# jzbontar/mc-cnn

Hardware: AMD Instinct MI355X
Metric: Mega-pixel-disparities/sec (cost-vol+CBCA+SGM) + end-to-end disp ms/pair (higher is better)
Workload: dtype f32; 1 GPU; KITTI 2012 fast, 370x1226 disp_max=228; H=370, W=1226, disp_max=228, feature_channels=64, params=kitti_fast, parallelism=one pair per GPU

## Files before the change

mc-cnn_amd/csrc/api.hip:

```cpp
#include "cbca_common.h"

#include <stdarg.h>
#include <algorithm>
#include <map>
#include <mutex>
#include <vector>

namespace mc {

int fill_nan(float *p, int64_t n, hipStream_t st);
int scale(const float *in, float *out, int64_t n, float s, hipStream_t st);
int transpose(const float *in, float *out, int64_t R, int64_t Cn, int64_t ldin, int64_t ldout, float s, hipStream_t st, int nt = -1);
int fix_border(float *vol, int D, int H, int W, int n, int direction, hipStream_t st);
int argmin_dhw(const float *vol, float *out, int D, int H, int W, int base1, hipStream_t st);
int outlier_detection(const float *d0, const float *d1, float *outlier, int H, int W, int disp_max, hipStream_t st);
int interpolate_occlusion(const float *d0, const float *outlier, float *out, int H, int W, hipStream_t st);
int interpolate_mismatch(const float *d0, const float *outlier, float *out, int H, int W, hipStream_t st);
int subpixel(const float *d0, const float *vol, float *out, int D, int H, int W, int64_t sd, int64_t sp, hipStream_t st);
int median2d(const float *img, float *out, int H, int W, int k, hipStream_t st);
int mean2d(const float *img, const float *kernel, float *out, int H, int W, int ks, float alpha2, hipStream_t st);
int normalize_forward(const float *in, float *norm, float *out, int N, int C, int H, int W, hipStream_t st);
int stereo_join_dhw(const float *fL, const float *fR, float *volL, float *volR, int C, int D, int H, int W, hipStream_t st);
int stereo_join_hwd(const float *fL, const float *fR, float *volL, float *volR, int C, int D, int ds, int H, int W, int n,
                    hipStream_t st);
int ad_tiled(const float *x0, const float *x1, float *vol, int D, int H, int W, int direction, hipStream_t st);
size_t census_scratch_bytes(int Cimg, int H, int W);
int census_sig(const float *x0, const float *x1, float *vol, void *scratch, int Cimg, int D, int H, int W, int direction,
               hipStream_t st);
int cross(const float *img, float *arms, int H, int W, int L1, float tau1, hipStream_t st);
int cbca(const float *x0c, const float *x1c, const float *vin, float *vout, int D, int H, int W, int direction, hipStream_t st);
size_t cbca_scratch_bytes(int H, int W);
int cbca_pack(const float *x0c, const float *x1c, void *scratch, int H, int W, hipStream_t st);
int cbca_if_overflow(const float *x0c, const float *x1c, const void *packed, const float *vin, float *vout, int D, int H, int W,
                     int direction, hipStream_t st);
int cbca_strips(const void *packed, const float *vin, float *vout, int D, int H, int W, int direction, int route,
               hipStream_t st, const CbcaCfg &cfg = CbcaCfg());
size_t cbca_plan_bytes(int D, int H, int W);
int cbca_tiles(const void *packed, const float *vin, float *vout, int D, int H, int W, int direction, int arm_class, int route,
               hipStream_t st, const CbcaCfg &cfg = CbcaCfg());
bool cbca_lean_fits(int D, int H, int W, size_t plan_bytes, bool two_pass = false, int rb = 0);
int cbca_classify(const void *packed, void *plan, size_t plan_bytes, int D, int H, int W, int direction, int route, int rb, int cap_limit,
                  hipStream_t st, bool two_pass = false, float cost_limit = 0);
int cbca_lean2x(const void *packed, const void *plan, size_t plan_bytes, const float *vin, float *vout, int D, int H, int W, int direction,
                int route, hipStream_t st, const CbcaCfg &cfg);
int cbca_lean(const void *packed, const void *plan, size_t plan_bytes, const float *vin, float *vout, int D, int H, int W, int direction,
              int route, hipStream_t st, const CbcaCfg &cfg);
size_t conv3x3_workspace_bytes(int Cin, int Cout);
int conv3x3(const float *in, const float *w, const float *bias, float *out, int N, int Cin, int Cout, int H, int W, int relu,
            void *workspace, hipStream_t st);
size_t fc_workspace_bytes(int C, int n_hidden, int H, int W);
int fc_stack(const float *featL, const float *featR, int C, int H, int W, int D, const float *const *weights,
             const float *const *biases, int n_layers, float *volL, float *volR, void *workspace, hipStream_t st);
size_t sgm_maps_bytes(int H, int W);
int sgm_prep(const float *x0, const float *x1, void *maps, int H, int W, float tau_so, hipStream_t st);
int sgm_contract_violations(const float *vol, int H, int W, int D, unsigned *count, hipStream_t st);
int sgm_sweeps(const float *const C[2], float *const out[2], float *const out2[2], float *const disp[2],
               const int direction[2], int nvol, int H, int W, int D, int ds, const void *maps, float pi1, float pi2,
               float alpha1, float q1, float q2, bool fused, unsigned drop_final, hipStream_t st);

static thread_local char g_err[512] = "";

void set_error(const char *fmt, ...)
{
	va_list ap;
	va_start(ap, fmt);
	vsnprintf(g_err, sizeof(g_err), fmt, ap);
	va_end(ap);
}

int check_launch(const char *what)
{
	const hipError_t e = hipPeekAtLastError();
	if (e != hipSuccess) {
		(void)hipGetLastError();
		set_error("%s: %s", what, hipGetErrorString(e));
		return (int)e;
	}
	return 0;
}

static bool dims_ok(int D, int H, int W) { return D >= 1 && H >= 1 && W >= 1 && (int64_t)D * H * W < ((int64_t)1 << 40); }

static void gaussian_fill(double sigma, float *k)
{
	const int kr = (int)ceil(sigma * 3);
	const int ks = kr * 2 + 1;
	for (int i = 1; i <= ks; ++i) {
		for (int j = 1; j <= ks; ++j) {
			const double y = (i - 1) - kr;
			const double x = (j - 1) - kr;
			k[(size_t)(i - 1) * ks + (j - 1)] = (float)exp(-(x * x + y * y) / (2 * sigma * sigma));
		}
	}
}
struct GaussianK { const float *data; size_t n; };
static int gaussian_cached(double sigma, GaussianK &out)
{
	static std::mutex mu;
	static std::map<double, GaussianK> cache;
	std::lock_guard<std::mutex> lk(mu);
	auto it = cache.find(sigma);
	if (it != cache.end()) { out = it->second; return 0; }
	const int kr = (int)ceil(sigma * 3);
	const int ks = kr * 2 + 1;
	float *k = nullptr;
	const hipError_t e = hipHostMalloc((void **)&k, (size_t)ks * ks * sizeof(float), hipHostMallocDefault);
	if (e != hipSuccess) {
		set_error("gaussian: hipHostMalloc: %s", hipGetErrorString(e));
		return (int)e;
	}
	gaussian_fill(sigma, k);
	out = GaussianK{k, (size_t)ks * ks};
	cache[sigma] = out;
	return 0;
}

static inline size_t align_up(size_t v, size_t a) { return (v + a - 1) / a * a; }

static inline bool packed_dims_ok(int H, int W)
{
	return (int64_t)H * W < ((int64_t)1 << 29) - 4096 && H < (1 << 23) - 64 && W < (1 << 23) - 256;
}

static int cbca_by_arms(const void *packed, const float *vin, float *vout, int D, int H, int W, int direction, int max_arm, hipStream_t st,
                        const CbcaCfg &cfg = CbcaCfg())
{
	if (max_arm >= 0 && max_arm <= 4) return cbca_tiles(packed, vin, vout, D, H, W, direction, 4, -1, st, cfg);
	if (cfg.planned) {
		int rc = cbca_tiles(packed, vin, vout, D, H, W, direction, 13, CR_PLANNED_TILE13, st, cfg);
		if (rc || cfg.lean_two_pass) return rc;
		return cbca_strips(packed, vin, vout, D, H, W, direction, CR_STRIP_IF_LIST, st, cfg);
	}
	int rc = cbca_tiles(packed, vin, vout, D, H, W, direction, 4, CR_TILE4, st, cfg);
	if (rc) return rc;
	if (max_arm < 0 || max_arm <= 13) {
		rc = cbca_tiles(packed, vin, vout, D, H, W, direction, 13, CR_TILE13, st, cfg);
		if (rc) return rc;
	}
	if (cfg.lean) {
		if (!cfg.lean_two_pass) {
			rc = cbca_lean(packed, cfg.plan, cfg.plan_bytes, vin, vout, D, H, W, direction, CR_STRIP, st, cfg);
			if (rc) return rc;
		}
		return cbca_strips(packed, vin, vout, D, H, W, direction, CR_STRIP_IF_NO_LIST, st, cfg);
	}
	return cbca_strips(packed, vin, vout, D, H, W, direction, max_arm > 13 ? CR_STRIP_OR_TILE13 : CR_STRIP, st, cfg);
}

struct Plan {
	int Dp;
	size_t maps, arms, pack, vol, img, gk;
	size_t cplan;
	int nplan;
	size_t total;
};

struct StageCounts { int cbca1, sgm, cbca2; bool active_after; };
static StageCounts stage_counts(const mc_params *p)
{
	StageCounts c;
	bool sm_active = p->sm_terminate != MC_SM_CNN;
	c.cbca1 = (sm_active && p->sm_skip != MC_SKIP_CBCA) ? p->cbca_i1 : 0;
	sm_active = sm_active && p->sm_terminate != MC_SM_CBCA1;
	c.sgm = (sm_active && p->sm_skip != MC_SKIP_SGM) ? p->sgm_i : 0;
	sm_active = sm_active && p->sm_terminate != MC_SM_SGM;
	c.cbca2 = (sm_active && p->sm_skip != MC_SKIP_CBCA) ? p->cbca_i2 : 0;
	sm_active = sm_active && p->sm_terminate != MC_SM_CBCA2;
	c.active_after = sm_active;
	return c;
}

static Plan make_plan(const mc_params *p, int D, int H, int W)
{
	Plan pl;
	pl.Dp = (D + 3) / 4 * 4;
	const size_t HW = (size_t)H * W;
	pl.maps = align_up(sgm_maps_bytes(H, W), 256);
	pl.arms = align_up(8 * HW * sizeof(float), 256);
	pl.pack = cbca_scratch_bytes(H, W);
	pl.vol = align_up((size_t)pl.Dp * HW * sizeof(float), 256);
	pl.img = align_up(HW * sizeof(float), 256);
	const int kr = (int)ceil(p->blur_sigma * 3);
	const int ks = 2 * kr + 1;
	pl.gk = align_up((size_t)ks * ks * sizeof(float), 256);
	const StageCounts sc = stage_counts(p);
	pl.cplan = (sc.cbca1 + sc.cbca2 >= 2 && p->L1 - 1 <= 13) ? align_up(cbca_plan_bytes(D, H, W), 256) : 0;
	pl.nplan = (p->left_only && !p->lr_check) ? 1 : 2;
	constexpr int NVOLS = 6;
	pl.total = pl.maps + pl.arms + pl.pack + NVOLS * pl.vol + 6 * pl.img + pl.gk + pl.nplan * pl.cplan;
	return pl;
}

struct StageTimer {
	bool on = false;
	hipStream_t st;
	std::vector<hipEvent_t> ev;
	std::vector<int> tag;
	void mark(int stage)
	{
		if (!on) return;
		hipEvent_t e;
		(void)hipEventCreate(&e);
		(void)hipEventRecord(e, st);
		ev.push_back(e);
		tag.push_back(stage);
	}
	void collect(float out[MC_N_STAGES])
	{
		for (int i = 0; i < MC_N_STAGES; ++i) out[i] = 0;
		if (!on || ev.empty()) return;
		(void)hipEventSynchronize(ev.back());
		for (size_t i = 1; i < ev.size(); ++i) {
			float ms = 0;
			(void)hipEventElapsedTime(&ms, ev[i - 1], ev[i]);
			if (tag[i] >= 0 && tag[i] < MC_N_STAGES) out[tag[i]] += ms;
		}
		for (auto e : ev) (void)hipEventDestroy(e);
		ev.clear();
	}
};
enum { ST_PREP = MC_STAGE_PREP, ST_JOIN = MC_STAGE_JOIN, ST_CBCA = MC_STAGE_CBCA, ST_LAYOUT = MC_STAGE_LAYOUT,
       ST_SGM = MC_STAGE_SGM, ST_ARGMIN = MC_STAGE_ARGMIN, ST_POST = MC_STAGE_POST };

static int predict_impl(const mc_params *p, const float *x0, const float *x1, const float *featL, const float *featR, int C,
                        const float *rawL, const float *rawR, int D, int H, int W, void *workspace, size_t workspace_bytes,
                        float *volL_out, float *volR_out, float *dispL0_out, float *dispR0_out, float *disp_out, hipStream_t st,
                        StageTimer &tm)
{
	MC_REQUIRE(p && x0 && x1 && disp_out && workspace, "mc_predict: null argument");
	MC_REQUIRE(dims_ok(D, H, W), "mc_predict: bad dims D=%d H=%d W=%d", D, H, W);
	MC_REQUIRE(D <= MC_SGM_MAX_D, "mc_predict: D=%d exceeds %d", D, MC_SGM_MAX_D);
	MC_REQUIRE((featL && featR && C >= 1) || (rawL && rawR), "mc_predict: need features or raw volumes");
	MC_REQUIRE(p->cbca_i1 >= 0 && p->cbca_i2 >= 0 && p->sgm_i >= 0, "mc_predict: negative iteration count");
	MC_REQUIRE(p->median_k % 2 == 1 && p->median_k <= 11, "mc_predict: median_k must be odd and <= 11");
	MC_REQUIRE(p->blur_sigma > 0, "mc_predict: blur_sigma must be > 0");
	MC_REQUIRE(p->sm_terminate >= 0 && p->sm_terminate <= MC_SM_BILATERAL && p->sm_skip >= 0 && p->sm_skip <= MC_SKIP_BILATERAL,
	           "mc_predict: bad sm_terminate / sm_skip");
	const bool from_feat = featL != nullptr;
	if (from_feat) MC_REQUIRE(p->border_n >= 0 && p->border_n < W, "mc_predict: border_n=%d out of range", p->border_n);
	if (from_feat) MC_REQUIRE(C <= MC_JOIN_MAX_C, "mc_predict: C=%d exceeds %d (adcensus.cu:1460)", C, MC_JOIN_MAX_C);
	const Plan pl = make_plan(p, D, H, W);
	MC_REQUIRE(workspace_bytes >= pl.total, "mc_predict: workspace %zu < %zu bytes", workspace_bytes, pl.total);
	MC_REQUIRE((uintptr_t)workspace % 256 == 0, "mc_predict: workspace must be 256-byte aligned");

	const int64_t HW = (int64_t)H * W;
	const int64_t V = (int64_t)D * HW;
	char *w = (char *)workspace;
	void *maps = w; w += pl.maps;
	float *x0c = (float *)w; float *x1c = x0c + 4 * HW; w += pl.arms;
	void *packed = w; w += pl.pack;
	float *bufA[2], *bufB[2];
	bufA[0] = (float *)w; w += pl.vol;
	bufA[1] = (float *)w; w += pl.vol;
	bufB[0] = (float *)w; w += pl.vol;
	bufB[1] = (float *)w; w += pl.vol;
	float *bufC[2];
	bufC[0] = (float *)w; w += pl.vol;
	bufC[1] = (float *)w; w += pl.vol;
	float *img[6];
	for (int i = 0; i < 6; ++i) { img[i] = (float *)w; w += pl.img; }
	float *gk = (float *)w; w += pl.gk;
	void *cplan[2] = {pl.cplan ? (void *)w : nullptr, (pl.cplan && pl.nplan > 1) ? (void *)(w + pl.cplan) : nullptr};
	int cplan_passes[2] = {0, 0};
	bool cplan_listed[2] = {false, false};
	const int Dp = pl.Dp;
	int rc;
#define RUN(call) do { rc = (call); if (rc) return rc; } while (0)

	const int direction[2] = {-1, 1};
	const StageCounts sc = stage_counts(p);
	const int n_cbca1 = sc.cbca1, n_sgm = sc.sgm, n_cbca2 = sc.cbca2;
	bool sm_active = sc.active_after;
	const bool use_cbca = (n_cbca1 + n_cbca2) > 0;
	tm.mark(-1);

	if (n_sgm > 0) RUN(sgm_prep(x0, x1, maps, H, W, p->tau_so, st));
	if (use_cbca) {
		RUN(cross(x0, x0c, H, W, p->L1, p->tau1, st));
		RUN(cross(x1, x1c, H, W, p->L1, p->tau1, st));
		RUN(cbca_pack(x0c, x1c, packed, H, W, st));
	}
	const int cbca_cap = p->L1 - 1;
	tm.mark(ST_PREP);

	const int ds = Dp;
	const float *cur[2];
	auto other = [&](int v) -> float * { return cur[v] == bufA[v] ? bufB[v] : bufA[v]; };
	bool hwd;
	const int nvol = (p->left_only && !p->lr_check && !volR_out && !dispR0_out) ? 1 : 2;
	auto cbca_iterations = [&](int n) -> int {
		const bool packed_ok = cbca_cap <= 254 && packed_dims_ok(H, W);
		for (int v = 0; v < nvol; ++v) {
			const bool planned = packed_ok && cplan[v] && cbca_cap > 4 && cbca_cap <= 13 && cbca_lean_fits(D, H, W, pl.cplan, true);
			if (planned && n > 0 && !cplan_listed[v]) {
				const int rc1 = cbca_classify(packed, cplan[v], pl.cplan, D, H, W, direction[v], CR_STRIP, 0, 0, st, true);
				if (rc1) return rc1;
				cplan_listed[v] = true;
			}
			for (int i = 0; i < n;) {
				float *dst = other(v);
				CbcaCfg cfg;
				cfg.plan = cplan[v];
				cfg.plan_bytes = pl.cplan;
				cfg.planned = planned;
				const bool two = planned && i + 1 < n;
				cfg.lean = cfg.lean_two_pass = two;
				float *mid = two ? bufC[v] : dst;
				for (int half = 0; half < (two ? 2 : 1); ++half) {
					cfg.plan_mode = cplan[v] ? (cplan_passes[v]++ == 0 ? 1 : 2) : 0;
					const float *src = half == 0 ? cur[v] : mid;
					float *to = (two && half == 0) ? mid : dst;
					const int rc2 = packed_ok ? cbca_by_arms(packed, src, to, D, H, W, direction[v], cbca_cap, st, cfg)
					                          : cbca(x0c, x1c, src, to, D, H, W, direction[v], st);
					if (rc2) return rc2;
				}
				if (two) {
					const int rc3 = cbca_lean2x(packed, cplan[v], pl.cplan, cur[v], dst, D, H, W, direction[v], CR_STRIP, st, cfg);
					if (rc3) return rc3;
				}
				cur[v] = dst;
				i += two ? 2 : 1;
			}
		}
		return 0;
	};
	const bool join_fits = (int64_t)W * ((D + 3) / 4 * 4) * 4 < ((int64_t)1 << 31) && ((int64_t)(C + 64) * HW + W) * 4 < ((int64_t)1 << 31);
	if (from_feat && n_cbca1 == 0 && n_sgm > 0 && join_fits) {
		RUN(stereo_join_hwd(featL, featR, bufA[0], bufA[1], C, D, ds, H, W, p->border_n, st));
		cur[0] = bufA[0]; cur[1] = bufA[1];
		hwd = true;
		tm.mark(ST_JOIN);
	} else {
		if (from_feat) {
			RUN(fill_nan(bufA[0], V, st));
			RUN(fill_nan(bufA[1], V, st));
			RUN(stereo_join_dhw(featL, featR, bufA[0], bufA[1], C, D, H, W, st));
			RUN(fix_border(bufA[0], D, H, W, p->border_n, -1, st));
			RUN(fix_border(bufA[1], D, H, W, p->border_n, 1, st));
			cur[0] = bufA[0]; cur[1] = bufA[1];
		} else {
			cur[0] = rawL; cur[1] = rawR;
		}
		hwd = false;
		tm.mark(ST_JOIN);
		RUN(cbca_iterations(n_cbca1));
		tm.mark(ST_CBCA);
	}

	float *dispv[2] = {img[0], img[1]};
	bool have_disp = false;
	if (n_sgm > 0) {
		if (!hwd) {
			for (int v = 0; v < nvol; ++v) {
				float *dst = other(v);
				RUN(transpose(cur[v], dst, D, HW, HW, ds, 1.0f, st));
				cur[v] = dst;
			}
			hwd = true;
			tm.mark(ST_LAYOUT);
		}
		for (int it = 0; it < n_sgm; ++it) {
			const float *Cv[2] = {cur[0], cur[1]};
			float *outv[2] = {other(0), other(1)};
			const bool am = (it == n_sgm - 1) && n_cbca2 == 0;
			const unsigned drop_final = (am && nvol == 2 && !volR_out) ? 2u : 0u;
			RUN(sgm_sweeps(Cv, outv, bufC, am ? dispv : nullptr, direction, nvol, H, W, D, ds, maps, p->pi1, p->pi2, p->alpha1,
			               p->sgm_q1, p->sgm_q2, true, drop_final, st));
			have_disp = am;
			cur[0] = outv[0]; cur[1] = outv[1];
		}
		tm.mark(ST_SGM);
		if (n_cbca2 > 0) {
			for (int v = 0; v < nvol; ++v) {
				float *dst = other(v);
				RUN(transpose(cur[v], dst, HW, D, ds, HW, 1.0f, st));
				cur[v] = dst;
			}
			hwd = false;
			tm.mark(ST_LAYOUT);
		}
	}
	if (!hwd) {
		RUN(cbca_iterations(n_cbca2));
		tm.mark(ST_CBCA);
	}

	MC_REQUIRE(have_disp || !hwd, "mc_predict: an (H,W,D) volume without its arg-min");
	if (!have_disp) {
		for (int v = 0; v < nvol; ++v) RUN(argmin_dhw(cur[v], dispv[v], D, H, W, 0, st));
	}
	float *vout[2] = {volL_out, volR_out};
	for (int v = 0; v < nvol; ++v) {
		if (!vout[v]) continue;
		if (hwd) RUN(transpose(cur[v], vout[v], HW, D, ds, HW, 1.0f, st));
		else RUN(scale(cur[v], vout[v], V, 1.0f, st));
	}
	if (dispL0_out) RUN(scale(dispv[0], dispL0_out, HW, 1.0f, st));
	if (dispR0_out) RUN(scale(dispv[1], dispR0_out, HW, 1.0f, st));
	tm.mark(ST_ARGMIN);

	float *d = dispv[0];
	float *outl = img[4];
	int nfree = 0;
	float *freeimg[3] = {img[2], img[3], img[5]};
	auto next = [&]() -> float * {
		float *r = freeimg[nfree % 3];
		if (r == d) r = freeimg[++nfree % 3];
		++nfree;
		return r;
	};
	if (p->lr_check) {
		RUN(outlier_detection(d, dispv[1], outl, H, W, D, st));
		if (sm_active && p->sm_skip != MC_SKIP_OCCLUSION) {
			float *o = next();
			RUN(interpolate_occlusion(d, outl, o, H, W, st));
			d = o;
		}
		sm_active = sm_active && p->sm_terminate != MC_SM_OCCLUSION;
		if (sm_active && p->sm_skip != MC_SKIP_OCCLUSION) {
			float *o = next();
			RUN(interpolate_mismatch(d, outl, o, H, W, st));
			d = o;
		}
		sm_active = sm_active && p->sm_terminate != MC_SM_MISMATCH;
	}
	if (sm_active && p->sm_skip != MC_SKIP_SUBPIXEL) {
		float *o = next();
		if (hwd) RUN(subpixel(d, cur[0], o, D, H, W, 1, ds, st));
		else RUN(subpixel(d, cur[0], o, D, H, W, HW, 1, st));
		d = o;
	}
	sm_active = sm_active && p->sm_terminate != MC_SM_SUBPIXEL;
	if (sm_active && p->sm_skip != MC_SKIP_MEDIAN) {
		float *o = next();
		RUN(median2d(d, o, H, W, p->median_k, st));
		d = o;
	}
	sm_active = sm_active && p->sm_terminate != MC_SM_MEDIAN;
	if (sm_active && p->sm_skip != MC_SKIP_BILATERAL) {
		GaussianK k;
		RUN(gaussian_cached(p->blur_sigma, k));
		const int ks = 2 * (int)ceil(p->blur_sigma * 3) + 1;
		const hipError_t e = hipMemcpyAsync(gk, k.data, k.n * sizeof(float), hipMemcpyHostToDevice, st);
		if (e != hipSuccess) {
			set_error("mc_predict: kernel upload: %s", hipGetErrorString(e));
			return (int)e;
		}
		RUN(mean2d(d, gk, disp_out, H, W, ks, p->blur_t, st));
	} else {
		RUN(scale(d, disp_out, HW, 1.0f, st));
	}
	tm.mark(ST_POST);
#undef RUN
	return 0;
}

}

using namespace mc;

extern "C" {

int mc_version(void) { return MC_ABI_VERSION; }
const char *mc_last_error(void) { return g_err; }

int mc_fill_nan(float *p, int64_t n, void *stream)
{
	MC_REQUIRE(p || n == 0, "mc_fill_nan: null pointer");
	MC_REQUIRE(n >= 0, "mc_fill_nan: negative size");
	return fill_nan(p, n, as_stream(stream));
}

int mc_stereo_join(const float *featL, const float *featR, float *volL, float *volR, int C, int D, int H, int W, void *stream)
{
	MC_REQUIRE(featL && featR && volL && volR, "mc_stereo_join: null pointer");
	MC_REQUIRE(dims_ok(D, H, W) && C >= 1, "mc_stereo_join: bad dims C=%d D=%d H=%d W=%d", C, D, H, W);
	MC_REQUIRE(C <= MC_JOIN_MAX_C, "mc_stereo_join: C=%d exceeds %d (adcensus.cu:1460)", C, MC_JOIN_MAX_C);
	MC_REQUIRE(D <= 65535, "mc_stereo_join: D too large");
	return stereo_join_dhw(featL, featR, volL, volR, C, D, H, W, as_stream(stream));
}

int mc_ad(const float *x0, const float *x1, float *vol, int D, int H, int W, int direction, void *stream)
{
	MC_REQUIRE(x0 && x1 && vol, "mc_ad: null pointer");
	MC_REQUIRE(dims_ok(D, H, W), "mc_ad: bad dims");
	MC_REQUIRE(direction == -1 || direction == 1, "mc_ad: direction must be -1 or 1");
	MC_REQUIRE(D <= 65535, "mc_ad: D too large");
	return ad_tiled(x0, x1, vol, D, H, W, direction, as_stream(stream));
}

size_t mc_census_scratch_bytes(int Cimg, int H, int W)
{
	if (Cimg < 1 || H < 1 || W < 1) return 0;
	return census_scratch_bytes(Cimg, H, W);
}

int mc_census_ws(const float *x0, const float *x1, float *vol, int Cimg, int D, int H, int W, int direction, void *scratch,
                 size_t scratch_bytes, void *stream)
{
	MC_REQUIRE(x0 && x1 && vol && scratch, "mc_census_ws: null pointer");
	MC_REQUIRE(dims_ok(D, H, W) && Cimg >= 1 && D <= 65535, "mc_census_ws: bad dims");
	MC_REQUIRE(direction == -1 || direction == 1, "mc_census_ws: direction must be -1 or 1");
	MC_REQUIRE(scratch_bytes >= census_scratch_bytes(Cimg, H, W), "mc_census_ws: scratch holds %zu bytes, needs %zu", scratch_bytes,
	           census_scratch_bytes(Cimg, H, W));
	MC_REQUIRE((uintptr_t)scratch % 4 == 0, "mc_census_ws: scratch must be 4-byte aligned");
	return census_sig(x0, x1, vol, scratch, Cimg, D, H, W, direction, as_stream(stream));
}

size_t mc_fc_stack_workspace_bytes(int C, int n_layers, int H, int W)
{
	if (C < 1 || n_layers < 2 || n_layers > 8 || H < 1 || W < 1) return 0;
	return fc_workspace_bytes(C, n_layers - 2, H, W);
}

int mc_fc_stack(const float *featL, const float *featR, int C, int H, int W, int D, const float *const *weights,
                const float *const *biases, const int *layer_out, int n_layers, float *volL, float *volR, void *workspace,
                size_t workspace_bytes, void *stream)
{
	MC_REQUIRE(featL && featR && weights && biases && layer_out && volL && volR && workspace, "mc_fc_stack: null pointer");
	MC_REQUIRE(dims_ok(D, H, W) && C >= 1, "mc_fc_stack: bad dims");
	MC_REQUIRE(n_layers >= 2 && n_layers <= 8, "mc_fc_stack: 2..8 layers supported");
	for (int l = 0; l < n_layers - 1; ++l)
		MC_REQUIRE(layer_out[l] == 384, "mc_fc_stack: hidden width %d not supported (nh2 = 384 in every preset, main.lua:77,124)",
		           layer_out[l]);
	MC_REQUIRE(layer_out[n_layers - 1] == 1, "mc_fc_stack: the last layer must have one output");
	for (int l = 0; l < n_layers; ++l) MC_REQUIRE(weights[l] && biases[l], "mc_fc_stack: null layer %d", l);
	MC_REQUIRE(workspace_bytes >= fc_workspace_bytes(C, n_layers - 2, H, W), "mc_fc_stack: workspace %zu < %zu bytes",
	           workspace_bytes, fc_workspace_bytes(C, n_layers - 2, H, W));
	MC_REQUIRE((uintptr_t)workspace % 16 == 0, "mc_fc_stack: workspace must be 16-byte aligned");
	MC_REQUIRE((int64_t)((H + 7) / 8) * ((W + 95) / 96) * D * 8 < ((int64_t)1 << 31), "mc_fc_stack: problem too large for one launch");
	return fc_stack(featL, featR, C, H, W, D, weights, biases, n_layers, volL, volR, workspace, as_stream(stream));
}

size_t mc_conv3x3_workspace_bytes(int Cin, int Cout)
{
	if (Cin < 1 || Cout < 1 || Cout > 128) return 0;
	return conv3x3_workspace_bytes(Cin, Cout);
}

int mc_conv3x3(const float *in, const float *weight, const float *bias, float *out, int N, int Cin, int Cout, int H, int W,
               int relu, void *workspace, size_t workspace_bytes, void *stream)
{
	MC_REQUIRE(in && weight && bias && out && workspace && in != out, "mc_conv3x3: bad pointers");
	MC_REQUIRE(N >= 1 && Cin >= 1 && Cout >= 1 && dims_ok(1, H, W), "mc_conv3x3: bad dims");
	MC_REQUIRE(Cout <= 128, "mc_conv3x3: Cout=%d exceeds 128 (the nets of main.lua:73-75, 120-122 use 64 and 112)", Cout);
	MC_REQUIRE((int64_t)(Cout > Cin ? Cout : Cin + 1) * H * W * 4 < (int64_t)0xFFFFFF00 && (int64_t)N * ((W + 31) / 32) * H < ((int64_t)1 << 31),
	           "mc_conv3x3: %d x %d x (%d -> %d channels) x %d images exceeds the kernel's 32-bit offsets", H, W, Cin, Cout, N);
	MC_REQUIRE(workspace_bytes >= conv3x3_workspace_bytes(Cin, Cout), "mc_conv3x3: workspace %zu < %zu bytes", workspace_bytes,
	           conv3x3_workspace_bytes(Cin, Cout));
	MC_REQUIRE((uintptr_t)workspace % 16 == 0, "mc_conv3x3: workspace must be 16-byte aligned");
	return conv3x3(in, weight, bias, out, N, Cin, Cout, H, W, relu, workspace, as_stream(stream));
}

int mc_fix_border(float *vol, int D, int H, int W, int n, int direction, void *stream)
{
	MC_REQUIRE(vol, "mc_fix_border: null pointer");
	MC_REQUIRE(dims_ok(D, H, W), "mc_fix_border: bad dims");
	MC_REQUIRE(n >= 0 && n < W, "mc_fix_border: n=%d out of range for W=%d", n, W);
	MC_REQUIRE(direction == -1 || direction == 1, "mc_fix_border: direction must be -1 or 1");
	return fix_border(vol, D, H, W, n, direction, as_stream(stream));
}

int mc_cross(const float *img, float *arms, int H, int W, int L1, float tau1, void *stream)
{
	MC_REQUIRE(img && arms, "mc_cross: null pointer");
	MC_REQUIRE(dims_ok(1, H, W), "mc_cross: bad dims");
	return cross(img, arms, H, W, L1, tau1, as_stream(stream));
}

int mc_cbca(const float *x0c, const float *x1c, const float *vol_in, float *vol_out, int D, int H, int W, int direction,
            void *stream)
{
	MC_REQUIRE(x0c && x1c && vol_in && vol_out, "mc_cbca: null pointer");
	MC_REQUIRE(vol_in != vol_out, "mc_cbca: in-place aggregation is not supported (the reference uses a tmp volume too)");
	MC_REQUIRE(dims_ok(D, H, W) && D <= 65535, "mc_cbca: bad dims");
	MC_REQUIRE(direction == -1 || direction == 1, "mc_cbca: direction must be -1 or 1");
	return cbca(x0c, x1c, vol_in, vol_out, D, H, W, direction, as_stream(stream));
}

size_t mc_cbca_scratch_bytes(int H, int W)
{
	if (H < 1 || W < 1) return 0;
	return cbca_scratch_bytes(H, W);
}

int mc_cbca_ws(const float *x0c, const float *x1c, const float *vol_in, float *vol_out, int D, int H, int W, int direction,
               void *scratch, size_t scratch_bytes, void *stream)
{
	MC_REQUIRE(x0c && x1c && vol_in && vol_out && scratch, "mc_cbca_ws: null pointer");
	MC_REQUIRE(vol_in != vol_out, "mc_cbca_ws: in-place aggregation is not supported (the reference uses a tmp volume too)");
	MC_REQUIRE(dims_ok(D, H, W) && D <= 65535 * 8, "mc_cbca_ws: bad dims");
	MC_REQUIRE(direction == -1 || direction == 1, "mc_cbca_ws: direction must be -1 or 1");
	MC_REQUIRE(scratch_bytes >= cbca_scratch_bytes(H, W), "mc_cbca_ws: scratch holds %zu bytes, needs %zu", scratch_bytes,
	           cbca_scratch_bytes(H, W));
	MC_REQUIRE((uintptr_t)scratch % 4 == 0, "mc_cbca_ws: scratch must be 4-byte aligned");
	hipStream_t st = as_stream(stream);
	if (!packed_dims_ok(H, W))
		return cbca(x0c, x1c, vol_in, vol_out, D, H, W, direction, st);
	int rc = cbca_pack(x0c, x1c, scratch, H, W, st);
	if (rc) return rc;
	rc = cbca_by_arms(scratch, vol_in, vol_out, D, H, W, direction, -1, st);
	if (rc) return rc;
	return cbca_if_overflow(x0c, x1c, scratch, vol_in, vol_out, D, H, W, direction, st);
}

size_t mc_cbca_plan_bytes(int D, int H, int W)
{
	if (!dims_ok(D, H, W)) return 0;
	return align_up(cbca_scratch_bytes(H, W), 256) - cbca_scratch_bytes(H, W) + cbca_plan_bytes(D, H, W);
}

int mc_cbca_ws_cfg(const float *x0c, const float *x1c, const float *vol_in, float *vol_out, int D, int H, int W, int direction,
                   void *scratch, size_t scratch_bytes, int rb, int nt, int d0, int nd, int form, void *stream)
{
	MC_REQUIRE(x0c && x1c && vol_in && vol_out && scratch, "mc_cbca_ws_cfg: null pointer");
	MC_REQUIRE(vol_in != vol_out, "mc_cbca_ws_cfg: in-place aggregation is not supported");
	MC_REQUIRE(dims_ok(D, H, W) && D <= 65535 * 8, "mc_cbca_ws_cfg: bad dims");
	MC_REQUIRE(direction == -1 || direction == 1, "mc_cbca_ws_cfg: direction must be -1 or 1");
	MC_REQUIRE(scratch_bytes >= cbca_scratch_bytes(H, W), "mc_cbca_ws_cfg: scratch holds %zu bytes, needs %zu", scratch_bytes,
	           cbca_scratch_bytes(H, W));
	MC_REQUIRE((uintptr_t)scratch % 4 == 0, "mc_cbca_ws_cfg: scratch must be 4-byte aligned");
	MC_REQUIRE(packed_dims_ok(H, W), "mc_cbca_ws_cfg: image too large for the packed-length kernels (32-bit plane offsets, 24-bit row indices)");
	MC_REQUIRE(rb >= 0 && rb <= 4096 && nt >= -1 && nt <= 1 && form >= 0 && form <= 11, "mc_cbca_ws_cfg: bad rb / nt / form");
	MC_REQUIRE(d0 >= 0 && nd >= 0 && (form >= 8 || d0 + nd <= D), "mc_cbca_ws_cfg: planes [%d, %d) outside the volume", d0, d0 + nd);
	hipStream_t st = as_stream(stream);
	int rc = cbca_pack(x0c, x1c, scratch, H, W, st);
	if (rc) return rc;
	CbcaCfg cfg;
	cfg.nt = nt; cfg.d0 = d0; cfg.nd = nd;
	if (form >= 10) {
		const size_t off = align_up(cbca_scratch_bytes(H, W), 256), pb = align_up(cbca_plan_bytes(D, H, W), 256);
		const size_t vb = (size_t)D * H * W * sizeof(float);
		MC_REQUIRE(scratch_bytes >= off + pb + vb, "mc_cbca_ws_cfg: scratch holds %zu bytes, needs %zu with the list and a volume", scratch_bytes, off + pb + vb);
		MC_REQUIRE((uintptr_t)scratch % 16 == 0, "mc_cbca_ws_cfg: scratch must be 16-byte aligned for the list");
		cfg.plan = (char *)scratch + off;
		cfg.plan_bytes = pb;
		cfg.lean_rb = rb;
		cfg.lean_two_pass = true;
		cfg.d0 = 0; cfg.nd = 0;
		float *mid = (float *)((char *)scratch + off + pb);
		const bool fits = cbca_lean_fits(D, H, W, pb, true, rb);
		if (fits && form == 10) {
			rc = cbca_classify(scratch, cfg.plan, cfg.plan_bytes, D, H, W, direction, CR_NOT_DIRECT, rb, 0, st, true, (float)d0);
			if (rc) return rc;
		}
		if (fits) {
			rc = cbca_lean2x(scratch, cfg.plan, cfg.plan_bytes, vol_in, vol_out, D, H, W, direction, CR_NOT_DIRECT, st, cfg);
			if (rc) return rc;
		}
		const int sroute = fits ? CR_NOT_DIRECT_IF_NO_LIST : CR_NOT_DIRECT;
		rc = cbca_strips(scratch, vol_in, mid, D, H, W, direction, sroute, st, cfg);
		if (rc) return rc;
		rc = cbca_strips(scratch, mid, vol_out, D, H, W, direction, sroute, st, cfg);
		if (rc) return rc;
		rc = cbca_if_overflow(x0c, x1c, scratch, vol_in, mid, D, H, W, direction, st);
		if (rc) return rc;
		return cbca_if_overflow(x0c, x1c, scratch, mid, vol_out, D, H, W, direction, st);
	}
	if (form >= 8) {
		const size_t off = align_up(cbca_scratch_bytes(H, W), 256), pb = cbca_plan_bytes(D, H, W);
		MC_REQUIRE(scratch_bytes >= off + pb, "mc_cbca_ws_cfg: scratch holds %zu bytes, needs %zu with the list", scratch_bytes, off + pb);
		MC_REQUIRE((uintptr_t)scratch % 16 == 0, "mc_cbca_ws_cfg: scratch must be 16-byte aligned for the list");
		MC_REQUIRE(cbca_lean_fits(D, H, W, pb), "mc_cbca_ws_cfg: volume too large for 32-bit list entries");
		cfg.plan = (char *)scratch + off;
		cfg.plan_bytes = pb;
		cfg.lean_rb = rb;
		cfg.lean_variant = d0; cfg.d0 = 0; cfg.nd = nd;
		if (form == 8) {
			rc = cbca_classify(scratch, cfg.plan, cfg.plan_bytes, D, H, W, direction, CR_NOT_DIRECT, rb, nd, st);
			if (rc) return rc;
		}
		rc = cbca_lean(scratch, cfg.plan, cfg.plan_bytes, vol_in, vol_out, D, H, W, direction, CR_NOT_DIRECT, st, cfg);
		if (rc) return rc;
		cfg.nd = 0;
		rc = cbca_strips(scratch, vol_in, vol_out, D, H, W, direction, CR_NOT_DIRECT_IF_NO_LIST, st, cfg);
		if (rc) return rc;
		return cbca_if_overflow(x0c, x1c, scratch, vol_in, vol_out, D, H, W, direction, st);
	}
	if (form >= 4) {
		const size_t off = align_up(cbca_scratch_bytes(H, W), 256);
		MC_REQUIRE(scratch_bytes >= off + cbca_plan_bytes(D, H, W), "mc_cbca_ws_cfg: scratch holds %zu bytes, needs %zu with the plan", scratch_bytes,
		           off + cbca_plan_bytes(D, H, W));
		MC_REQUIRE((uintptr_t)scratch % 16 == 0, "mc_cbca_ws_cfg: scratch must be 16-byte aligned for the plan");
		cfg.plan = (char *)scratch + off;
		cfg.plan_mode = form <= 5 ? 1 : 2;
		const bool shortarm = form == 4 || form == 6;
		return cbca_tiles(scratch, vol_in, vol_out, D, H, W, direction, shortarm ? 4 : 13, shortarm ? CR_ARMS_LE4 : CR_ARMS_LE13, st, cfg);
	}
	if (form >= 2) {
		cfg.variant = rb;
		return cbca_tiles(scratch, vol_in, vol_out, D, H, W, direction, form == 2 ? 4 : 13, form == 2 ? CR_ARMS_LE4 : CR_ARMS_LE13, st, cfg);
	}
	cfg.rb = rb;
	rc = form == 1 ? cbca_strips(scratch, vol_in, vol_out, D, H, W, direction, CR_NOT_DIRECT, st, cfg)
	               : cbca_by_arms(scratch, vol_in, vol_out, D, H, W, direction, -1, st, cfg);
	if (rc) return rc;
	return cbca_if_overflow(x0c, x1c, scratch, vol_in, vol_out, D, H, W, direction, st);
}

int mc_transpose_cfg(const float *in, float *out, int64_t rows, int64_t cols, int64_t ldin, int64_t ldout, float scale_, int nt,
                     void *stream)
{
	MC_REQUIRE(in && out && in != out, "mc_transpose_cfg: bad pointers");
	MC_REQUIRE(rows >= 1 && cols >= 1 && ldin >= cols && ldout >= rows, "mc_transpose_cfg: bad dims");
	MC_REQUIRE(nt >= -1 && nt <= 1, "mc_transpose_cfg: bad nt");
	return transpose(in, out, rows, cols, ldin, ldout, scale_, as_stream(stream), nt);
}


int mc_sgm2_contract_violations(const float *in_hwd, int H, int W, int D, unsigned *count, void *stream)
{
	MC_REQUIRE(in_hwd && count, "mc_sgm2_contract_violations: null pointer");
	MC_REQUIRE(dims_ok(D, H, W), "mc_sgm2_contract_violations: bad dims");
	return sgm_contract_violations(in_hwd, H, W, D, count, as_stream(stream));
}

size_t mc_sgm2_tmp_bytes(int H, int W, int D)
{
	(void)D;
	if (H < 1 || W < 1) return 0;
	return sgm_maps_bytes(H, W);
}

int mc_sgm2(const float *x0, const float *x1, const float *in_hwd, float *out_hwd, void *tmp, size_t tmp_bytes, int H, int W,
            int D, float pi1, float pi2, float tau_so, float alpha1, float sgm_q1, float sgm_q2, int direction, void *stream)
{
	MC_REQUIRE(x0 && x1 && in_hwd && out_hwd && tmp, "mc_sgm2: null pointer");
	MC_REQUIRE(dims_ok(D, H, W), "mc_sgm2: bad dims");
	MC_REQUIRE(D <= MC_SGM_MAX_D, "mc_sgm2: D=%d exceeds %d", D, MC_SGM_MAX_D);
	MC_REQUIRE(direction == -1 || direction == 1, "mc_sgm2: direction must be -1 or 1");
	MC_REQUIRE(tmp_bytes >= sgm_maps_bytes(H, W), "mc_sgm2: tmp holds %zu bytes, needs %zu", tmp_bytes, sgm_maps_bytes(H, W));
	MC_REQUIRE(in_hwd != out_hwd, "mc_sgm2: input and output must differ");
	hipStream_t st = as_stream(stream);
	int rc = sgm_prep(x0, x1, tmp, H, W, tau_so, st);
	if (rc) return rc;
	const float *Cv[2] = {in_hwd, in_hwd};
	float *outv[2] = {out_hwd, out_hwd};
	const int dirv[2] = {direction, direction};
	return sgm_sweeps(Cv, outv, nullptr, nullptr, dirv, 1, H, W, D, D, tmp, pi1, pi2, alpha1, sgm_q1, sgm_q2, false, 0u, st);
}

int mc_dhw_to_hwd(const float *in, float *out, int D, int H, int W, void *stream)
{
	MC_REQUIRE(in && out && in != out, "mc_dhw_to_hwd: bad pointers");
	MC_REQUIRE(dims_ok(D, H, W), "mc_dhw_to_hwd: bad dims");
	return transpose(in, out, D, (int64_t)H * W, (int64_t)H * W, D, 1.0f, as_stream(stream));
}

int mc_hwd_to_dhw(const float *in, float *out, int D, int H, int W, float scale_, void *stream)
{
	MC_REQUIRE(in && out && in != out, "mc_hwd_to_dhw: bad pointers");
	MC_REQUIRE(dims_ok(D, H, W), "mc_hwd_to_dhw: bad dims");
	return transpose(in, out, (int64_t)H * W, D, D, (int64_t)H * W, scale_, as_stream(stream));
}

int mc_scale(const float *in, float *out, int64_t n, float s, void *stream)
{
	MC_REQUIRE((in && out) || n == 0, "mc_scale: null pointer");
	MC_REQUIRE(n >= 0, "mc_scale: negative size");
	return scale(in, out, n, s, as_stream(stream));
}

int mc_argmin(const float *vol, float *disp, int D, int H, int W, void *stream)
{
	MC_REQUIRE(vol && disp, "mc_argmin: null pointer");
	MC_REQUIRE(dims_ok(D, H, W), "mc_argmin: bad dims");
	return argmin_dhw(vol, disp, D, H, W, 0, as_stream(stream));
}

int mc_spatial_argmin(const float *vol, float *out, int D, int H, int W, void *stream)
{
	MC_REQUIRE(vol && out, "mc_spatial_argmin: null pointer");
	MC_REQUIRE(dims_ok(D, H, W), "mc_spatial_argmin: bad dims");
	return argmin_dhw(vol, out, D, H, W, 1, as_stream(stream));
}

int mc_outlier_detection(const float *d0, const float *d1, float *outlier, int H, int W, int disp_max, void *stream)
{
	MC_REQUIRE(d0 && d1 && outlier, "mc_outlier_detection: null pointer");
	MC_REQUIRE(dims_ok(1, H, W) && disp_max >= 0, "mc_outlier_detection: bad dims");
	return outlier_detection(d0, d1, outlier, H, W, disp_max, as_stream(stream));
}

int mc_interpolate_occlusion(const float *d0, const float *outlier, float *out, int H, int W, void *stream)
{
	MC_REQUIRE(d0 && outlier && out && out != d0, "mc_interpolate_occlusion: bad pointers");
	MC_REQUIRE(dims_ok(1, H, W), "mc_interpolate_occlusion: bad dims");
	return interpolate_occlusion(d0, outlier, out, H, W, as_stream(stream));
}

int mc_interpolate_mismatch(const float *d0, const float *outlier, float *out, int H, int W, void *stream)
{
	MC_REQUIRE(d0 && outlier && out && out != d0, "mc_interpolate_mismatch: bad pointers");
	MC_REQUIRE(dims_ok(1, H, W), "mc_interpolate_mismatch: bad dims");
	return interpolate_mismatch(d0, outlier, out, H, W, as_stream(stream));
}

int mc_subpixel_enchancement(const float *d0, const float *vol, float *out, int D, int H, int W, void *stream)
{
	MC_REQUIRE(d0 && vol && out, "mc_subpixel_enchancement: null pointer");
	MC_REQUIRE(dims_ok(D, H, W), "mc_subpixel_enchancement: bad dims");
	return subpixel(d0, vol, out, D, H, W, (int64_t)H * W, 1, as_stream(stream));
}

int mc_median2d(const float *img, float *out, int H, int W, int kernel_size, void *stream)
{
	MC_REQUIRE(img && out && img != out, "mc_median2d: bad pointers");
	MC_REQUIRE(dims_ok(1, H, W), "mc_median2d: bad dims");
	MC_REQUIRE(kernel_size % 2 == 1 && kernel_size >= 1 && kernel_size <= 11,
	           "mc_median2d: kernel_size must be odd and <= 11 (adcensus.cu:1601-1602)");
	return median2d(img, out, H, W, kernel_size, as_stream(stream));
}

int mc_mean2d(const float *img, const float *kernel, float *out, int H, int W, int ks, float alpha2, void *stream)
{
	MC_REQUIRE(img && kernel && out && img != out, "mc_mean2d: bad pointers");
	MC_REQUIRE(dims_ok(1, H, W), "mc_mean2d: bad dims");
	MC_REQUIRE(ks % 2 == 1 && ks >= 1, "mc_mean2d: kernel size must be odd (adcensus.cu:1269)");
	return mean2d(img, kernel, out, H, W, ks, alpha2, as_stream(stream));
}

int mc_gaussian_host(double sigma, float *host_kernel, int capacity)
{
	MC_REQUIRE(sigma > 0, "mc_gaussian_host: sigma must be > 0");
	const int ks = 2 * (int)ceil(sigma * 3) + 1;
	if (host_kernel) {
		MC_REQUIRE(capacity >= ks * ks, "mc_gaussian_host: capacity %d < %d", capacity, ks * ks);
		gaussian_fill(sigma, host_kernel);
	}
	return ks;
}

int mc_normalize_forward(const float *in, float *norm, float *out, int N, int C, int H, int W, void *stream)
{
	MC_REQUIRE(in && out, "mc_normalize_forward: null pointer");
	MC_REQUIRE(N >= 1 && C >= 1 && dims_ok(1, H, W), "mc_normalize_forward: bad dims");
	return normalize_forward(in, norm, out, N, C, H, W, as_stream(stream));
}

size_t mc_predict_workspace_bytes(const mc_params *p, int C, int D, int H, int W)
{
	(void)C;
	if (!p || !dims_ok(D, H, W) || !(p->blur_sigma > 0)) return 0;
	return make_plan(p, D, H, W).total;
}

int mc_predict(const mc_params *p, const float *x0, const float *x1, const float *featL, const float *featR, int C,
               const float *rawL, const float *rawR, int D, int H, int W, void *workspace, size_t workspace_bytes,
               float *volL_out, float *volR_out, float *dispL0_out, float *dispR0_out, float *disp_out, void *stream)
{
	StageTimer tm;
	return predict_impl(p, x0, x1, featL, featR, C, rawL, rawR, D, H, W, workspace, workspace_bytes, volL_out, volR_out,
	                    dispL0_out, dispR0_out, disp_out, as_stream(stream), tm);
}

int mc_predict_timed(const mc_params *p, const float *x0, const float *x1, const float *featL, const float *featR, int C,
                     const float *rawL, const float *rawR, int D, int H, int W, void *workspace, size_t workspace_bytes,
                     float *disp_out, void *stream, float *stage_ms)
{
	StageTimer tm;
	tm.on = stage_ms != nullptr;
	tm.st = as_stream(stream);
	const int rc = predict_impl(p, x0, x1, featL, featR, C, rawL, rawR, D, H, W, workspace, workspace_bytes, nullptr, nullptr,
	                            nullptr, nullptr, disp_out, tm.st, tm);
	if (stage_ms) tm.collect(stage_ms);
	return rc;
}

}
```

mc-cnn_amd/csrc/sgm.hip:

```cpp
#include "mc_common.h"

#define MC_SGM_VOL_AUX 2
#define MC_SGM_ST_AUX MC_SGM_VOL_AUX

namespace mc {

constexpr int SGM_PADW = 520;

struct SgmPassArgs {
	const float *C[2];
	const float *accin[2];
	const float *accin2[2];
	float *out[2];
	float *out2[2];
	float *disp[2];
	int drop_out[2];
	int direction[2];
	int nvol;
	int H, W, D, ds;
	const uint8_t *cls0;
	int64_t cls_plane;
	const uint8_t *win;
	int Wm;
	float P1[3], P2[3], P1a[3];
};

__device__ __forceinline__ int cls_of(float v, float tau) { return v < tau ? 0 : (v > tau ? 2 : 1); }

__global__ void __launch_bounds__(256) sgm_prep_kernel(const float *__restrict__ x0, const float *__restrict__ x1,
                                                       uint8_t *__restrict__ cls0, uint8_t *__restrict__ win,
                                                       int H, int W, int Wm, int64_t cls_plane, float tau_so)
{
	const int64_t id = (int64_t)blockIdx.x * blockDim.x + threadIdx.x;
	const int64_t total = (int64_t)4 * H * Wm;
	if (id >= total) return;
	const int i = (int)(id % Wm);
	const int y = (int)((id / Wm) % H);
	const int r = (int)(id / ((int64_t)Wm * H));
	const int dx = r == 0 ? 1 : (r == 1 ? -1 : 0);
	const int dy = r == 2 ? 1 : (r == 3 ? -1 : 0);
	const bool yok = (y - dy >= 0) && (y - dy < H);

	if (i < W) {
		const int x = i;
		int c = 1;
		if (yok && x - dx >= 0 && x - dx < W) {
			c = cls_of(fabsf(x0[y * W + x] - x0[(y - dy) * W + x - dx]), tau_so);
		}
		cls0[(int64_t)r * cls_plane + (int64_t)y * W + x] = (uint8_t)c;
	}
	const int s = i - SGM_PADW;
	unsigned asc = 0, desc = 0;
#pragma unroll
	for (int k = 0; k < 4; ++k) {
		const int xx = s + k;
		float D2 = 10.0f;
		if (yok && xx >= 0 && xx < W && xx - dx >= 0 && xx - dx < W) {
			D2 = fabsf(x1[y * W + xx] - x1[(y - dy) * W + xx - dx]);
		}
		const unsigned c = (unsigned)cls_of(D2, tau_so);
		asc |= c << (2 * k);
		desc |= c << (2 * (3 - k));
	}
	win[((int64_t)(0 * 4 + r) * H + y) * Wm + i] = (uint8_t)asc;
	win[((int64_t)(1 * 4 + r) * H + y) * Wm + i] = (uint8_t)desc;
}

typedef unsigned uint4v __attribute__((ext_vector_type(4)));

template <int VPL, int NACC>
struct StepData {
	float c[VPL];
	float a[NACC > 0 ? VPL : 1];
	float a2[NACC > 1 ? VPL : 1];
	unsigned pk;
	unsigned a0;
};


__device__ __forceinline__ float vmin2(float a, float b)
{
	float r;
	asm("v_min_f32 %0, %1, %2" : "=v"(r) : "v"(a), "v"(b));
	return r;
}
__device__ __forceinline__ float vmin3(float a, float b, float c)
{
	float r;
	asm("v_min3_f32 %0, %1, %2, %3" : "=v"(r) : "v"(a), "v"(b), "v"(c));
	return r;
}
__device__ __forceinline__ float wave_min_q(float v)
{
	float r;
	asm volatile("s_nop 1\n\tv_min_f32_dpp %1, %1, %1 quad_perm:[1,0,3,2] row_mask:0xf bank_mask:0xf\n\t"
	             "s_nop 1\n\tv_min_f32_dpp %1, %1, %1 quad_perm:[2,3,0,1] row_mask:0xf bank_mask:0xf\n\t"
	             "s_nop 1\n\tv_min_f32_dpp %1, %1, %1 row_half_mirror row_mask:0xf bank_mask:0xf\n\t"
	             "s_nop 1\n\tv_min_f32_dpp %1, %1, %1 row_mirror row_mask:0xf bank_mask:0xf\n\t"
	             "s_nop 1\n\tv_min_f32_dpp %1, %1, %1 row_bcast:15 row_mask:0xa bank_mask:0xf\n\t"
	             "s_nop 1\n\tv_min_f32_dpp %1, %1, %1 row_bcast:31 row_mask:0xc bank_mask:0xf\n\t"
	             "s_nop 0\n\tv_readlane_b32 %0, %1, 63"
	             : "=s"(r), "+v"(v));
	return r;
}

__device__ __forceinline__ __amdgpu_buffer_rsrc_t pixel_rsrc(const float *base, int64_t elem_off, int bytes)
{
	return __builtin_amdgcn_make_buffer_rsrc((void *)(base + elem_off), 0, bytes, 0x00020000);
}

template <int DIRN, int VPL, int MODE, bool ARGMIN, bool VEC, int U, bool DUAL, bool FAR>
__device__ __forceinline__ void sgm_line(const SgmPassArgs &A, int wave)
{
	constexpr int NACC = MODE == 0 ? 0 : (MODE == 3 ? 2 : 1);
	const int lane = threadIdx.x & 63;
	const int H = A.H, W = A.W, D = A.D, ds = A.ds, Wm = A.Wm;
	const int nlines = DIRN <= 1 ? H : W;
	const int nsteps = DIRN <= 1 ? W : H;
	const int nw = A.nvol * nlines;
	bool second = false;
	if (DUAL) {
		if (wave >= 2 * nw) return;
		second = wave >= nw;
		if (second) wave -= nw;
	} else if (wave >= nw) {
		return;
	}
	const int dirn = (DUAL && second) ? 1 : DIRN;
	const int v = wave / nlines;
	const int line = wave - v * nlines;
	const int direction = A.direction[v];
	const float *__restrict__ Cp = A.C[v];
	const float *__restrict__ Ain = A.accin[v];
	const float *__restrict__ Ain2 = A.accin2[v];
	float *__restrict__ Out = (DUAL && second) ? A.out2[v] : A.out[v];
	float *__restrict__ Disp = A.disp[v];
	const bool drop = A.drop_out[v];

	const int x0s = dirn == 0 ? 0 : (dirn == 1 ? W - 1 : line);
	const int y0s = dirn == 2 ? 0 : (dirn == 3 ? H - 1 : line);
	const int sx = dirn == 0 ? 1 : (dirn == 1 ? -1 : 0);
	const int sy = dirn == 2 ? 1 : (dirn == 3 ? -1 : 0);

	const int dbase = VPL * lane;
	const uint8_t *__restrict__ cls0 = A.cls0 + (int64_t)dirn * A.cls_plane;
	constexpr int WBIAS = 1024;
	const uint8_t *__restrict__ win = A.win + ((int64_t)((direction > 0 ? 0 : 1) * 4 + dirn) * H) * Wm + SGM_PADW - WBIAS;
	const int woff = (direction > 0 ? dbase : -dbase - 3) + WBIAS;
	const int wq = direction > 0 ? 4 : -4;
	const int run_bytes = (VEC ? ds : D) * 4;

	const float INF = __builtin_inff();
	const float P1mid = A.P1[1], P2mid = A.P2[1], P1amid = A.P1a[1];
	const float P1lo = A.P1[0], P2lo = A.P2[0], P1alo = A.P1a[0];
	const float P1hi = A.P1[2], P2hi = A.P2[2], P1ahi = A.P1a[2];

	const int last = nsteps - 1;
	const int pix0 = y0s * W + x0s, dp = sy * W + sx;
	const int minpix = dp > 0 ? pix0 : pix0 + last * dp;
	const unsigned c1v = (unsigned)(dp * ds * 4);
	const unsigned c0v = dp > 0 ? 0u : (unsigned)last * (unsigned)(-dp * ds * 4);
	const unsigned span = (unsigned)last * (unsigned)((dp > 0 ? dp : -dp) * ds * 4) + (unsigned)run_bytes;
	constexpr unsigned OOBV = 0x80000000u;
	const __amdgpu_buffer_rsrc_t rC = pixel_rsrc(Cp, (int64_t)minpix * ds, FAR ? 0 : span);
	const __amdgpu_buffer_rsrc_t rA = pixel_rsrc(NACC >= 1 ? Ain : Cp, (int64_t)minpix * ds, FAR ? 0 : span);
	const __amdgpu_buffer_rsrc_t rA2 = pixel_rsrc(NACC >= 2 ? Ain2 : Cp, (int64_t)minpix * ds, FAR ? 0 : span);
	const __amdgpu_buffer_rsrc_t rO = pixel_rsrc(Out, (int64_t)minpix * ds, (FAR || drop) ? 0 : span);
	const __amdgpu_buffer_rsrc_t rW = __builtin_amdgcn_make_buffer_rsrc((void *)win, 0, H * Wm + 2 * WBIAS + 64, 0x00020000);
	const int w0 = y0s * Wm + x0s, dw = sy * Wm + sx;
	const __amdgpu_buffer_rsrc_t rCls = __builtin_amdgcn_make_buffer_rsrc((void *)cls0, 0, H * W, 0x00020000);
	const __amdgpu_buffer_rsrc_t rDisp = pixel_rsrc(ARGMIN ? Disp : Out, 0, H * W * 4);
	unsigned lane_off[VEC ? VPL / 4 : VPL];
#pragma unroll
	for (int q = 0; q < (VEC ? VPL / 4 : VPL); ++q) {
		const unsigned b = (unsigned)(dbase + (VEC ? 4 * q : q)) * 4u;
		lane_off[q] = (FAR || b < (unsigned)run_bytes) ? b : OOBV;
	}
	const unsigned lane0_off = lane == 0 ? 0u : OOBV;

	auto load_run = [&](float (&dst)[VPL], const float *base, const __amdgpu_buffer_rsrc_t &rs, unsigned so, int64_t pix) {
		const __amdgpu_buffer_rsrc_t r = FAR ? pixel_rsrc(base, pix * ds, run_bytes) : rs;
		const unsigned soff = FAR ? 0u : so;
		if (VEC) {
#pragma unroll
			for (int q = 0; q < VPL / 4; ++q) {
				const uint4v t = __builtin_amdgcn_raw_buffer_load_b128(r, lane_off[q], soff, MC_SGM_VOL_AUX);
				dst[4 * q + 0] = __uint_as_float(t.x); dst[4 * q + 1] = __uint_as_float(t.y);
				dst[4 * q + 2] = __uint_as_float(t.z); dst[4 * q + 3] = __uint_as_float(t.w);
			}
		} else {
#pragma unroll
			for (int j = 0; j < VPL; ++j) dst[j] = __uint_as_float(__builtin_amdgcn_raw_buffer_load_b32(r, lane_off[j], soff, 0));
		}
	};

	auto load_step = [&](StepData<VPL, NACC> &sd, int s) {
		const unsigned so = c0v + (unsigned)s * c1v;
		const int64_t pix = FAR ? (int64_t)(y0s + s * sy) * W + (x0s + s * sx) : 0;
		load_run(sd.c, Cp, rC, so, pix);
		if constexpr (NACC >= 1) load_run(sd.a, Ain, rA, so, pix);
		if constexpr (NACC >= 2) load_run(sd.a2, Ain2, rA2, so, pix);
		unsigned pk = 0;
		const unsigned sw = (unsigned)(w0 + s * dw);
#pragma unroll
		for (int q = 0; q < VPL / 4; ++q) pk |= (unsigned)__builtin_amdgcn_raw_buffer_load_b8(rW, woff + q * wq, sw, 0) << (8 * q);
		sd.pk = pk;
		sd.a0 = __builtin_amdgcn_raw_buffer_load_b8(rCls, 0, (unsigned)(pix0 + s * dp), 0);
	};

	auto store_step = [&](const float (&o)[VPL], int s) {
		const int64_t pix = FAR ? (int64_t)(y0s + s * sy) * W + (x0s + s * sx) : 0;
		const __amdgpu_buffer_rsrc_t r = FAR ? pixel_rsrc(Out, pix * ds, drop ? 0 : run_bytes) : rO;
		const unsigned soff = FAR ? 0u : c0v + (unsigned)s * c1v;
		if (VEC) {
#pragma unroll
			for (int q = 0; q < VPL / 4; ++q) {
				uint4v t;
				t.x = __float_as_uint(o[4 * q + 0]); t.y = __float_as_uint(o[4 * q + 1]);
				t.z = __float_as_uint(o[4 * q + 2]); t.w = __float_as_uint(o[4 * q + 3]);
				__builtin_amdgcn_raw_buffer_store_b128(t, r, lane_off[q], soff, MC_SGM_ST_AUX);
			}
		} else {
#pragma unroll
			for (int j = 0; j < VPL; ++j) __builtin_amdgcn_raw_buffer_store_b32(__float_as_uint(o[j]), r, lane_off[j], soff, 0);
		}
		if (ARGMIN) {
			float best = INF;
			int bi = 0;
#pragma unroll
			for (int j = 0; j < VPL; ++j) {
				if (dbase + j < D && o[j] < best) {
					best = o[j];
					bi = dbase + j;
				}
			}
			const float mall = wave_min_q(best);
			const unsigned long long cand = __ballot(best == mall && best < INF);
			const int f = __builtin_ffsll((long long)cand);
			const int got = __builtin_amdgcn_readlane(bi, (f - 1) & 63);
			const int idx = f ? got : 0;
			__builtin_amdgcn_raw_buffer_store_b32(__float_as_uint((float)idx), rDisp, lane0_off, (unsigned)(pix0 + s * dp) * 4u, 0);
		}
	};

	float prev[VPL];
	float m = 0.0f;
#pragma unroll
	for (int j = 0; j < VPL; ++j) prev[j] = 0.0f;

	float P1midv = P1mid, P2midv = P2mid, P1amidv = P1amid, INFv = INF;
	asm volatile("" : "+v"(P1midv), "+v"(P2midv), "+v"(P1amidv), "+v"(INFv));
	const float zadd = (DUAL && second) ? -0.0f : 0.0f;

	auto process = [&](const StepData<VPL, NACC> &sd, int s, float *keep = nullptr) {
		float val[VPL], o[VPL];
		const int a0 = __builtin_amdgcn_readfirstlane((int)sd.a0);
		const int amatch = a0 == 1 ? 3 : a0;
		float P1x, P2x, P1ax = 0.0f;
		if (DIRN >= 2)
			asm("s_cmp_eq_u32 %3, 0\n\ts_cselect_b32 %0, %4, %5\n\ts_cselect_b32 %1, %6, %7\n\ts_cselect_b32 %2, %8, %9"
			    : "=s"(P1x), "=s"(P2x), "=s"(P1ax)
			    : "s"(a0), "s"(P1lo), "s"(P1hi), "s"(P2lo), "s"(P2hi), "s"(P1alo), "s"(P1ahi)
			    : "scc");
		else
			asm("s_cmp_eq_u32 %2, 0\n\ts_cselect_b32 %0, %3, %4\n\ts_cselect_b32 %1, %5, %6"
			    : "=s"(P1x), "=s"(P2x)
			    : "s"(a0), "s"(P1lo), "s"(P1hi), "s"(P2lo), "s"(P2hi)
			    : "scc");
		const float down = lane_from_below(prev[VPL - 1], INF);
		const float up = lane_from_above(prev[0], INF);
#pragma unroll
		for (int j = 0; j < VPL; ++j) {
			const int b = (sd.pk >> (2 * j)) & 3;
			const bool match = b == amatch;
			const float P2 = match ? P2x : P2midv;
			const float P1 = match ? P1x : P1midv;
			const float P1a = match ? P1ax : P1amidv;
			const float pm = j > 0 ? prev[j > 0 ? j - 1 : 0] : down;
			const float pp = j < VPL - 1 ? prev[j < VPL - 1 ? j + 1 : 0] : up;
			float cost;
			asm("v_min_f32 %0, %1, %2\n\tv_min3_f32 %0, %0, %3, %4"
			    : "=&v"(cost)
			    : "v"(prev[j]), "v"(m + P2), "v"(pm + (DIRN == 2 ? P1a : P1)), "v"(pp + (DIRN == 3 ? P1a : P1)));
			val[j] = (sd.c[j] + cost) - m;
		}
		if (s == 0) {
			asm volatile("; border step");
#pragma unroll
			for (int j = 0; j < VPL; ++j) val[j] = sd.c[j];
		}
		float q[VPL];
#pragma unroll
		for (int j = 0; j < VPL; ++j) {
			if (MODE == 0) o[j] = val[j] + zadd;
			else if (MODE == 1) o[j] = sd.a[j] + val[j];
			else if (MODE == 2) o[j] = (sd.a[j] + val[j]) * 0.25f;
			else o[j] = (sd.a[j] + sd.a2[j]) + val[j];
			q[j] = vmin2(val[j], INFv);
		}
#pragma unroll
		for (int j = 0; j < VPL; ++j) prev[j] = (dbase + j < D) ? q[j] : INFv;
		float nm = vmin3(prev[0], prev[1], prev[2]);
#pragma unroll
		for (int j = 3; j < VPL; j += 2) nm = j + 1 < VPL ? vmin3(nm, prev[j], prev[j + 1]) : vmin2(nm, prev[j]);
		m = wave_min_q(nm);
		if (keep) {
#pragma unroll
			for (int j = 0; j < VPL; ++j) keep[j] = o[j];
		} else {
			store_step(o, s);
		}
	};

	StepData<VPL, NACC> ring[U];
#pragma unroll
	for (int u = 0; u < U; ++u) load_step(ring[u], u < last ? u : last);

	int g = 0;
	constexpr int SB = (DIRN <= 1 && !ARGMIN && U % 4 == 0) ? 4 : 1;
	constexpr int LB = (DIRN <= 1 && U % 4 == 0) ? 4 : 1;
	float obuf[SB][VPL];
	for (; g + U <= nsteps; g += U) {
#pragma unroll
		for (int u = 0; u < U; ++u) {
			const int s = g + u;
			__builtin_amdgcn_sched_barrier(0);
			if (SB > 1) {
				process(ring[u], s, obuf[u % SB]);
				if (u % SB == SB - 1) {
#pragma unroll
					for (int k = 0; k < SB; ++k) store_step(obuf[k], s - (SB - 1) + k);
				}
			} else {
				process(ring[u], s);
			}
			if (u % LB == LB - 1) {
#pragma unroll
				for (int k = 0; k < LB; ++k) {
					const int sn = s - (LB - 1) + k + U;
					load_step(ring[u - (LB - 1) + k], sn < last ? sn : last);
				}
			}
		}
	}
#pragma unroll
	for (int u = 0; u < U; ++u) {
		if (g + u < nsteps) process(ring[u], g + u);
	}
}

template <int DIRN, int VPL, int MODE, bool ARGMIN, bool VEC, int U, bool DUAL, bool FAR>
__global__ void __launch_bounds__(256) sgm_pass_kernel(const SgmPassArgs A)
{
	sgm_line<DIRN, VPL, MODE, ARGMIN, VEC, U, DUAL, FAR>(A, __builtin_amdgcn_readfirstlane((int)((blockIdx.x * blockDim.x + threadIdx.x) >> 6)));
}


__global__ void __launch_bounds__(256) sgm_contract_kernel(const float *__restrict__ vol, int64_t pixels, int D, unsigned *__restrict__ count)
{
	const int64_t p = (int64_t)blockIdx.x * blockDim.x + threadIdx.x;
	bool bad = false;
	if (p < pixels) {
		const float *v = vol + p * D;
		bad = !(fabsf(v[0]) < __builtin_inff());
		bool seen_nan = false;
		for (int d = 0; d < D; ++d) {
			const bool isn = v[d] != v[d];
			bad = bad || (seen_nan && !isn);
			seen_nan = seen_nan || isn;
		}
	}
	const unsigned long long b = __ballot(bad);
	if ((threadIdx.x & 63) == 0 && b) atomicAdd(count, (unsigned)__builtin_popcountll(b));
}

int sgm_contract_violations(const float *vol, int H, int W, int D, unsigned *count, hipStream_t st)
{
	const int64_t pixels = (int64_t)H * W;
	hipError_t e = hipMemsetAsync(count, 0, sizeof(unsigned), st);
	if (e != hipSuccess) {
		set_error("mc_sgm2_contract_violations: hipMemsetAsync: %s", hipGetErrorString(e));
		return (int)e;
	}
	hipLaunchKernelGGL(sgm_contract_kernel, dim3(cdiv(pixels, 256)), dim3(256), 0, st, vol, pixels, D, count);
	return check_launch("sgm_contract");
}

size_t sgm_maps_bytes(int H, int W)
{
	const size_t Wm = (size_t)W + 2 * SGM_PADW;
	const size_t plane = ((size_t)H * W + 3 + 4) / 4 * 4;
	size_t b = 4 * plane + (size_t)8 * H * Wm;
	return (b + 255) & ~(size_t)255;
}

int sgm_prep(const float *x0, const float *x1, void *maps, int H, int W, float tau_so, hipStream_t st)
{
	const int Wm = W + 2 * SGM_PADW;
	const size_t plane = ((size_t)H * W + 3 + 4) / 4 * 4;
	uint8_t *cls0 = (uint8_t *)maps;
	uint8_t *win = cls0 + 4 * plane;
	const int64_t total = (int64_t)4 * H * Wm;
	hipLaunchKernelGGL(sgm_prep_kernel, dim3(cdiv(total, 256)), dim3(256), 0, st, x0, x1, cls0, win, H, W, Wm, (int64_t)plane,
	                   tau_so);
	return check_launch("sgm_prep");
}

constexpr int SGM_U_H = 8, SGM_U_UP = 16;
constexpr int SGM_U_DOWN = 16;

template <int DIRN, int MODE, bool ARGMIN, bool DUAL>
static void launch_pass(const SgmPassArgs &A, bool vec, hipStream_t st)
{
	const int nlines = DIRN <= 1 ? A.H : A.W;
	const int waves = A.nvol * nlines * (DUAL ? 2 : 1);
	const dim3 grid(cdiv(waves, 4)), block(256);
	const int U = DIRN == 2 ? SGM_U_DOWN : (DIRN == 3 ? SGM_U_UP : SGM_U_H);
	constexpr bool SCALAR = MODE == 1;
#define MC_SGM_GO(VPL_, VEC_, U_) \
	hipLaunchKernelGGL((sgm_pass_kernel<DIRN, VPL_, MODE, ARGMIN, VEC_, U_, DUAL, false>), grid, block, 0, st, A)
#define MC_SGM_GO_FAR(VPL_, VEC_, U_) \
	hipLaunchKernelGGL((sgm_pass_kernel<DIRN, VPL_, MODE, ARGMIN, VEC_, U_, DUAL, true>), grid, block, 0, st, A)
	const bool far = (int64_t)A.H * A.W * A.ds * 4 >= ((int64_t)1 << 31);
	if (!vec) {
		if constexpr (SCALAR) {
			if (far) { if (A.D <= 256) MC_SGM_GO_FAR(4, false, 4); else MC_SGM_GO_FAR(8, false, 2); }
			else { if (A.D <= 256) MC_SGM_GO(4, false, 4); else MC_SGM_GO(8, false, 2); }
		}
	} else if (far) {
		if (A.D <= 256) MC_SGM_GO_FAR(4, true, 4); else MC_SGM_GO_FAR(8, true, 4);
	} else if (A.D <= 256) {
		if (U == 16) MC_SGM_GO(4, true, 16); else if (U == 8) MC_SGM_GO(4, true, 8); else MC_SGM_GO(4, true, 4);
	} else {
		if (U >= 8) MC_SGM_GO(8, true, 8); else MC_SGM_GO(8, true, 4);
	}
#undef MC_SGM_GO_FAR
#undef MC_SGM_GO
}


int sgm_sweeps(const float *const C[2], float *const out[2], float *const out2[2], float *const disp[2],
               const int direction[2], int nvol, int H, int W, int D, int ds, const void *maps, float pi1, float pi2,
               float alpha1, float q1, float q2, bool fused, unsigned drop_final, hipStream_t st)
{
	MC_REQUIRE((int64_t)H * W < ((int64_t)1 << 29) && (int64_t)W * ds * 4 < ((int64_t)1 << 31), "sgm: image %dx%d (pixel stride %d) exceeds the sweeps' 32-bit line arithmetic", H, W, ds);
	SgmPassArgs A;
	for (int v = 0; v < 2; ++v) {
		const int k = v < nvol ? v : 0;
		A.C[v] = C[k];
		A.accin[v] = out[k];
		A.accin2[v] = out2 ? out2[k] : nullptr;
		A.out[v] = out[k];
		A.out2[v] = out2 ? out2[k] : nullptr;
		A.disp[v] = disp ? disp[k] : nullptr;
		A.direction[v] = direction[k];
		A.drop_out[v] = 0;
	}
	A.nvol = nvol;
	A.H = H; A.W = W; A.D = D; A.ds = ds;
	A.Wm = W + 2 * SGM_PADW;
	A.cls0 = (const uint8_t *)maps;
	A.cls_plane = (int64_t)(((size_t)H * W + 3 + 4) / 4 * 4);
	A.win = A.cls0 + 4 * A.cls_plane;
	A.P1[0] = pi1; A.P2[0] = pi2;
	A.P1[1] = pi1 / q1; A.P2[1] = pi2 / q1;
	A.P1[2] = pi1 / (q1 * q2); A.P2[2] = pi2 / (q1 * q2);
	for (int k = 0; k < 3; ++k) A.P1a[k] = A.P1[k] / alpha1;

	bool vec = (ds % 4 == 0);
	for (int v = 0; v < nvol; ++v) {
		vec = vec && ((uintptr_t)C[v] % 16 == 0) && ((uintptr_t)out[v] % 16 == 0);
		if (out2) vec = vec && ((uintptr_t)out2[v] % 16 == 0);
	}
	const bool am = fused && disp && disp[0];
	if (!fused) {
		launch_pass<0, 1, false, false>(A, vec, st);
		launch_pass<1, 1, false, false>(A, vec, st);
		launch_pass<2, 1, false, false>(A, vec, st);
		launch_pass<3, 1, false, false>(A, vec, st);
	} else {
		MC_REQUIRE(out2 && vec, "sgm: the fused sweeps need the second direction's scratch and 16-byte aligned volumes with ds %% 4 == 0");
		launch_pass<0, 0, false, true>(A, vec, st);
		launch_pass<2, 3, false, false>(A, vec, st);
		for (int v = 0; v < nvol; ++v) A.drop_out[v] = (drop_final >> v) & 1;
		if (am) launch_pass<3, 2, true, false>(A, vec, st);
		else launch_pass<3, 2, false, false>(A, vec, st);
	}
	return check_launch("sgm_pass");
}

}
```

mc-cnn_amd/csrc/stereo_join.hip:

```cpp
#include "mc_common.h"
#include <type_traits>

namespace mc {

constexpr int JD_PX = 64, JD_D = 32, JD_CK = 16, JD_RW = JD_PX + JD_D;

__global__ void __launch_bounds__(256) join_dhw_kernel(const float *__restrict__ fL, const float *__restrict__ fR,
                                                       float *__restrict__ volL, float *__restrict__ volR, int C, int D, int H, int W)
{
	__shared__ float Ls[JD_CK][JD_PX];
	__shared__ float Rs[JD_CK][JD_RW];
	const int tid = threadIdx.x, xi = tid & 63, dg = tid >> 6;
	const int x0 = blockIdx.x * JD_PX, y = blockIdx.y, d0 = blockIdx.z * JD_D;
	const int64_t HW = (int64_t)H * W;
	const float *__restrict__ rowL = fL + (int64_t)y * W;
	const float *__restrict__ rowR = fR + (int64_t)y * W;
	const int r0 = x0 - d0 - (JD_D - 1);
	float sum[8];
#pragma unroll
	for (int k = 0; k < 8; ++k) sum[k] = 0.0f;
	for (int c0 = 0; c0 < C; c0 += JD_CK) {
		__syncthreads();
		for (int e = tid; e < JD_CK * JD_PX; e += 256) {
			const int c = e / JD_PX, i = e % JD_PX;
			Ls[c][i] = (c0 + c < C && x0 + i < W) ? rowL[(int64_t)(c0 + c) * HW + x0 + i] : 0.0f;
		}
		for (int e = tid; e < JD_CK * JD_RW; e += 256) {
			const int c = e / JD_RW, j = e % JD_RW;
			const int xr = r0 + j;
			Rs[c][j] = (c0 + c < C && xr >= 0 && xr < W) ? rowR[(int64_t)(c0 + c) * HW + xr] : 0.0f;
		}
		__syncthreads();
		const int nc = min(JD_CK, C - c0);
		for (int c = 0; c < nc; ++c) {
			const float l = -Ls[c][xi];
#pragma unroll
			for (int k = 0; k < 8; ++k) sum[k] = fmaf(l, Rs[c][xi + (JD_D - 1) - (dg * 8 + k)], sum[k]);
		}
	}
	const int x = x0 + xi;
	if (x >= W) return;
#pragma unroll
	for (int k = 0; k < 8; ++k) {
		const int d = d0 + dg * 8 + k;
		if (d < D && x - d >= 0) {
			const int64_t id = (int64_t)d * HW + (int64_t)y * W + x;
			volL[id] = sum[k];
			volR[id - d] = sum[k];
		}
	}
}

int stereo_join_dhw(const float *fL, const float *fR, float *volL, float *volR, int C, int D, int H, int W, hipStream_t st)
{
	hipLaunchKernelGGL(join_dhw_kernel, dim3(cdiv(W, JD_PX), H, cdiv(D, JD_D)), dim3(256), 0, st, fL, fR, volL, volR, C, D, H, W);
	return check_launch("stereo_join");
}

typedef float floatx16 __attribute__((ext_vector_type(16)));
typedef unsigned cb_u4_t __attribute__((ext_vector_type(4)));

template <int KSTEPS>
__global__ void __launch_bounds__(256) join_mfma_kernel(const float *__restrict__ fL, const float *__restrict__ fR,
                                                        float *__restrict__ volL, float *__restrict__ volR, int C, int D,
                                                        int ds, int H, int W, int tiles_per_row)
{
	__shared__ float T[4][32 * 33];
	const int lane = threadIdx.x & 63;
	const int wid = threadIdx.x >> 6;
	const int b = blockIdx.x;
	const int xcd = b & 7, k = b >> 3;
	const int blocks_per_row = (tiles_per_row + 3) >> 2;
	const int y = (k / blocks_per_row) * 8 + xcd;
	const int tile = (k % blocks_per_row) * 4 + wid;
	if (y >= H || tile >= tiles_per_row) return;

	const int64_t HW = (int64_t)H * W;
	const float *__restrict__ fA = fL + (int64_t)y * W;
	const float *__restrict__ fB = fR + (int64_t)y * W;
	const int p0 = tile * 32;
	const int nl = lane & 31, kh = lane >> 5;
	const bool real_tile = p0 < W;
	float *Tw = T[wid];

	const unsigned feat_bytes = (unsigned)(((int64_t)(C - 1) * HW + W) * 4);
	const __amdgpu_buffer_rsrc_t rA = __builtin_amdgcn_make_buffer_rsrc((void *)fA, 0, feat_bytes, 0x00020000);
	const __amdgpu_buffer_rsrc_t rB = __builtin_amdgcn_make_buffer_rsrc((void *)fB, 0, feat_bytes, 0x00020000);
	const unsigned pair_bytes = (unsigned)(2 * HW * 4);
	const unsigned OOBF = 0x80000000u;
	float a[KSTEPS];
	{
		const int px = p0 + nl;
		const unsigned vo = (real_tile && px < W) ? (unsigned)((int64_t)kh * HW + px) * 4u : OOBF;
#pragma unroll
		for (int kk = 0; kk < KSTEPS; ++kk) {
			const int c = 2 * kk + kh;
			const float v = __uint_as_float(__builtin_amdgcn_raw_buffer_load_b32(rA, c < C ? vo : OOBF, kk * pair_bytes, 0));
			a[kk] = -v;
		}
	}
	const float NANV = __builtin_nanf("");
	const int nJ = (D + 30) / 32 + 1;

	auto load_b = [&](float (&bv)[KSTEPS], int J) {
		const int qx = p0 - 32 * J + nl;
		const bool qin = real_tile && qx >= 0 && qx < W;
		const unsigned vo = qin ? (unsigned)((int64_t)kh * HW + qx) * 4u : OOBF;
#pragma unroll
		for (int kk = 0; kk < KSTEPS; ++kk) {
			const int c = 2 * kk + kh;
			bv[kk] = __uint_as_float(__builtin_amdgcn_raw_buffer_load_b32(rB, c < C ? vo : OOBF, kk * pair_bytes, 0));
		}
	};

	const int row_bytes = W * ds * 4;
	const __amdgpu_buffer_rsrc_t rowL = __builtin_amdgcn_make_buffer_rsrc((void *)(volL + (int64_t)y * W * ds), 0, row_bytes, 0x00020000);
	const __amdgpu_buffer_rsrc_t rowR = __builtin_amdgcn_make_buffer_rsrc((void *)(volR + (int64_t)y * W * ds), 0, row_bytes, 0x00020000);

	float bcur[KSTEPS], bnxt[KSTEPS];
	load_b(bcur, 0);
	for (int J = 0; J < nJ; ++J) {
		const int q0 = p0 - 32 * J;
		if (J + 1 < nJ) load_b(bnxt, J + 1);
		floatx16 acc;
#pragma unroll
		for (int i = 0; i < 16; ++i) acc[i] = 0.0f;
		if (real_tile && q0 + 31 >= 0) {
#pragma unroll
			for (int kk = 0; kk < KSTEPS; ++kk) acc = __builtin_amdgcn_mfma_f32_32x32x2f32(a[kk], bcur[kk], acc, 0, 0, 0);
		}
		const int qn = q0 + nl;
		const bool qok = qn >= 0 && qn < W;
		if (real_tile) {
			const int dJ = 32 * J - nl;
			int off = (p0 + 4 * kh) * ds + 4 * kh + dJ;
#pragma unroll
			for (int i = 0; i < 16; ++i) {
				const int m = (i & 3) + 8 * (i >> 2) + 4 * kh;
				const int d = m + dJ;
				const bool ok = p0 + m < W && d >= 0 && d < D;
				const int mo = (i & 3) + 8 * (i >> 2);
				__builtin_amdgcn_raw_buffer_store_b32(__float_as_uint(qok ? acc[i] : NANV), rowL,
				                                      ok ? (unsigned)(off + mo * (ds + 1)) * 4u : 0x80000000u, 0, 0);
			}
		}
#pragma unroll
		for (int i = 0; i < 16; ++i) {
			const int m = (i & 3) + 8 * (i >> 2) + 4 * kh;
			Tw[m * 33 + nl] = acc[i];
		}
		{
			const int mL = nl;
			const bool pin = p0 + mL < W;
			const int offR = (q0 + kh) * ds + mL - kh + 32 * J;
#pragma unroll
			for (int i = 0; i < 16; ++i) {
				const int n = 2 * i + kh;
				const int xr = q0 + n;
				const int d = mL - n + 32 * J;
				const bool ok = xr >= 0 && xr < W && d >= 0 && d < D;
				const float v = Tw[mL * 33 + n];
				__builtin_amdgcn_raw_buffer_store_b32(__float_as_uint(pin ? v : NANV), rowR,
				                                      ok ? (unsigned)(offR + 2 * i * (ds - 1)) * 4u : 0x80000000u, 0, 0);
			}
		}
#pragma unroll
		for (int kk = 0; kk < KSTEPS; ++kk) bcur[kk] = bnxt[kk];
	}
}

#define MC_JOIN_STORE_AUX 2

template <int KSTEPS, int SIDE, int NT>
__device__ __forceinline__ void join_owner_tiles(const float *__restrict__ fL, const float *__restrict__ fR, float *__restrict__ vol,
                                                 int C, int D, int ds, int H, int W, int y, int tile0, float *__restrict__ rings)
{
	const int lane = threadIdx.x & 63;
	const int nl = lane & 31, kh = lane >> 5;
	const int64_t HW = (int64_t)H * W;
	const unsigned feat_bytes = (unsigned)(((int64_t)(C - 1) * HW + W) * 4);
	const __amdgpu_buffer_rsrc_t rA = __builtin_amdgcn_make_buffer_rsrc((void *)(fL + (int64_t)y * W), 0, feat_bytes, 0x00020000);
	const __amdgpu_buffer_rsrc_t rB = __builtin_amdgcn_make_buffer_rsrc((void *)(fR + (int64_t)y * W), 0, feat_bytes, 0x00020000);
	const unsigned pair_bytes = (unsigned)(2 * HW * 4);
	const unsigned OOBF = 0x80000000u;
	const float NANV = __builtin_nanf("");
	auto load_tile = [&](float (&v)[KSTEPS], const __amdgpu_buffer_rsrc_t &r, int p0, bool negate) {
		const int px = p0 + nl;
		const unsigned vo = (px >= 0 && px < W) ? (unsigned)((int64_t)kh * HW + px) * 4u : OOBF;
#pragma unroll
		for (int kk = 0; kk < KSTEPS; ++kk) {
			const float t = __uint_as_float(__builtin_amdgcn_raw_buffer_load_b32(r, vo + (unsigned)kk * pair_bytes, 0, 0));
			v[kk] = negate ? -t : t;
		}
	};
	auto load_partner = [&](float (&v)[KSTEPS], int T) { load_tile(v, SIDE == 0 ? rB : rA, 32 * T, false); };
	float own[NT][KSTEPS], pa[KSTEPS], pb[KSTEPS];
#pragma unroll
	for (int t = 0; t < NT; ++t) load_tile(own[t], SIDE == 0 ? rA : rB, 32 * (tile0 + t), true);
	const int nJ = (D + 30) / 32 + 1;
	const int nsteps = nJ + NT - 1;
	auto partner_of = [&](int s) { return SIDE == 0 ? tile0 + NT - 1 - s : tile0 + s; };
	load_partner(pa, partner_of(0));

	const int wbase = 4 * kh - nl;
	const int wrow = SIDE == 0 ? 4 * kh * 64 : nl * 64;

	const int fp = lane & 7;
	const int row_floats = W * ds;
	const __amdgpu_buffer_rsrc_t rrow = __builtin_amdgcn_make_buffer_rsrc((void *)(vol + (int64_t)y * row_floats), 0, row_floats * 4, 0x00020000);
	const int row_mis = (int)(((int64_t)y * row_floats) & 31);
	int fd0[NT][4];
	unsigned fgo[NT][4];
#pragma unroll
	for (int t = 0; t < NT; ++t) {
#pragma unroll
		for (int pass = 0; pass < 4; ++pass) {
			const int px = 32 * (tile0 + t) + pass * 8 + (lane >> 3);
			const int fo = pass * 8 + (lane >> 3);
			const int a_o = (row_mis + px * ds) & 31;
			const int c_o = SIDE == 0 ? fo : 31 - fo;
			const int kl = ((c_o + a_o - 63 + 64) >> 5) - 2 + 1;
			fd0[t][pass] = 32 * kl - a_o + 4 * fp;
			fgo[t][pass] = px < W ? (unsigned)(px * ds) * 4u : OOBF;
		}
	}
	auto tile_product = [&](int t, const float (&part)[KSTEPS], int p0, floatx16 &acc) {
#pragma unroll
		for (int i = 0; i < 16; ++i) acc[i] = 0.0f;
		const bool any_in = SIDE == 0 ? (p0 + 31 >= 0) : (p0 < W);
		if (any_in) {
#pragma unroll
			for (int kk = 0; kk < KSTEPS; ++kk)
				acc = SIDE == 0 ? __builtin_amdgcn_mfma_f32_32x32x2f32(own[t][kk], part[kk], acc, 0, 0, 0)
				                : __builtin_amdgcn_mfma_f32_32x32x2f32(part[kk], own[t][kk], acc, 0, 0, 0);
		}
	};
	auto tile_store = [&](int t, int J, int p0, const floatx16 &acc) {
		float *__restrict__ ring = rings + t * (32 * 64);
		const int jbit = (J & 1) << 5;
		const bool interior = J >= 1 && 32 * J + 31 < D && (SIDE == 0 ? p0 >= 0 : p0 + 31 < W);
		if (interior) {
#pragma unroll
			for (int i = 0; i < 16; ++i) {
				const int mc = (i & 3) + 8 * (i >> 2);
				ring[wrow + (SIDE == 0 ? mc * 64 : 0) + (((wbase + mc) & 63) ^ jbit)] = acc[i];
			}
		} else {
#pragma unroll
			for (int i = 0; i < 16; ++i) {
				const int mc = (i & 3) + 8 * (i >> 2);
				const int d = wbase + mc + 32 * J;
				const int po = SIDE == 0 ? p0 + nl : p0 + mc + 4 * kh;
				const bool pin = SIDE == 0 ? po >= 0 : po < W;
				if (d >= 0 && d < D) ring[wrow + (SIDE == 0 ? mc * 64 : 0) + (((wbase + mc) & 63) ^ jbit)] = pin ? acc[i] : NANV;
			}
		}
		const bool last = J + 1 == nJ;
#pragma unroll
		for (int pass = 0; pass < 4; ++pass) {
			const int d0 = fd0[t][pass] + 32 * J;
			const int fro = (pass * 8 + (lane >> 3)) * 64;
			const float4 v = *(const float4 *)(ring + fro + (d0 & 63));
			__builtin_amdgcn_raw_buffer_store_b128((cb_u4_t){__float_as_uint(v.x), __float_as_uint(v.y), __float_as_uint(v.z), __float_as_uint(v.w)},
			                                       rrow, ((unsigned)d0 < (unsigned)ds) ? fgo[t][pass] + (unsigned)d0 * 4u : OOBF, 0, MC_JOIN_STORE_AUX);
			if (last) {
				const int d1 = d0 + 32;
				const float4 u = *(const float4 *)(ring + fro + (d1 & 63));
				__builtin_amdgcn_raw_buffer_store_b128((cb_u4_t){__float_as_uint(u.x), __float_as_uint(u.y), __float_as_uint(u.z), __float_as_uint(u.w)},
				                                       rrow, ((unsigned)d1 < (unsigned)ds) ? fgo[t][pass] + (unsigned)d1 * 4u : OOBF, 0, MC_JOIN_STORE_AUX);
			}
		}
	};
	auto do_step = [&](int s, const float (&part)[KSTEPS]) {
		const int T = partner_of(s);
		floatx16 acc[NT];
#pragma unroll
		for (int t = 0; t < NT; ++t) {
			const int J = SIDE == 0 ? tile0 + t - T : T - tile0 - t;
			if (J >= 0 && J < nJ) { tile_product(t, part, 32 * T, acc[0]); tile_store(t, J, 32 * T, acc[0]); }
		}
	};
	for (int s = 0; s < nsteps; s += 2) {
		load_partner(pb, partner_of(s + 1));
		do_step(s, pa);
		load_partner(pa, partner_of(s + 2));
		if (s + 1 < nsteps) do_step(s + 1, pb);
	}
}

#define MC_JOIN_NT 2
#define MC_JOIN_WPB 4
template <int KSTEPS, int NT = MC_JOIN_NT>
__global__ void __launch_bounds__(64 * MC_JOIN_WPB) join_owner_kernel(const float *__restrict__ fL, const float *__restrict__ fR,
                                                         float *__restrict__ volL, float *__restrict__ volR, int C, int D, int ds,
                                                         int H, int W, int pairs_per_row)
{
	__shared__ __attribute__((aligned(16))) float rings[MC_JOIN_WPB][NT * 32 * 64];
	const int wid = __builtin_amdgcn_readfirstlane(threadIdx.x >> 6);
	const int b = blockIdx.x;
	const int xcd = b & 7, k = b >> 3;
	const int blocks_per_row = (2 * pairs_per_row + MC_JOIN_WPB - 1) / MC_JOIN_WPB;
	const int y = (k / blocks_per_row) * 8 + xcd;
	const int w = (k % blocks_per_row) * MC_JOIN_WPB + wid;
	if (y >= H || w >= 2 * pairs_per_row) return;
	if (w < pairs_per_row) join_owner_tiles<KSTEPS, 0, NT>(fL, fR, volL, C, D, ds, H, W, y, NT * w, rings[wid]);
	else join_owner_tiles<KSTEPS, 1, NT>(fL, fR, volR, C, D, ds, H, W, y, NT * (w - pairs_per_row), rings[wid]);
}

__global__ void __launch_bounds__(256) fix_border_hwd_kernel(float *__restrict__ vol, int D, int ds, int H, int W, int n,
                                                             int direction)
{
	const int lane = threadIdx.x & 63;
	const int64_t w = ((int64_t)blockIdx.x * blockDim.x + threadIdx.x) >> 6;
	if (w >= (int64_t)H * n) return;
	const int y = (int)(w / n), i = (int)(w % n) + 1;
	const int dst = direction < 0 ? W - i : i - 1;
	const int src = direction < 0 ? W - (n + 1) : n;
	const float *s = vol + ((int64_t)y * W + src) * ds;
	float *t = vol + ((int64_t)y * W + dst) * ds;
	for (int d = lane; d < D; d += 64) t[d] = s[d];
}

int stereo_join_hwd(const float *fL, const float *fR, float *volL, float *volR, int C, int D, int ds, int H, int W, int n,
                    hipStream_t st)
{
	const int rows8 = (H + 7) / 8;
	const int ks = (C + 1) / 2;
	const dim3 block(256);
	MC_REQUIRE(ds % 4 == 0 && (uintptr_t)volL % 16 == 0 && (uintptr_t)volR % 16 == 0,
	           "stereo_join_hwd: the volumes must be 16-byte aligned with a pixel stride ds %% 4 == 0 (ds = %d)", ds);
	if (ks <= 32) {
		const int tiles_own = ((W + 31) / 32 + MC_JOIN_NT - 1) / MC_JOIN_NT;
		const dim3 grid_o((unsigned)(rows8 * ((2 * tiles_own + MC_JOIN_WPB - 1) / MC_JOIN_WPB) * 8)), block_o(64 * MC_JOIN_WPB);
		if (ks <= 8) hipLaunchKernelGGL((join_owner_kernel<8>), grid_o, block_o, 0, st, fL, fR, volL, volR, C, D, ds, H, W, tiles_own);
		else if (ks <= 16) hipLaunchKernelGGL((join_owner_kernel<16>), grid_o, block_o, 0, st, fL, fR, volL, volR, C, D, ds, H, W, tiles_own);
		else hipLaunchKernelGGL((join_owner_kernel<32>), grid_o, block_o, 0, st, fL, fR, volL, volR, C, D, ds, H, W, tiles_own);
		int rc = check_launch("stereo_join_hwd (owner tiles)");
		if (rc || n <= 0) return rc;
		hipLaunchKernelGGL(fix_border_hwd_kernel, dim3(cdiv((int64_t)H * n * 64, 256)), block, 0, st, volL, D, ds, H, W, n, -1);
		hipLaunchKernelGGL(fix_border_hwd_kernel, dim3(cdiv((int64_t)H * n * 64, 256)), block, 0, st, volR, D, ds, H, W, n, 1);
		return check_launch("fix_border_hwd");
	}
	const int tiles = (W + D - 1 + 31) / 32;
	const int blocks_per_row = (tiles + 3) / 4;
	const dim3 grid((unsigned)(rows8 * blocks_per_row * 8));
#define MC_JOIN_LAUNCH(KS)                                                                                                  \
	do {                                                                                                                    \
		hipLaunchKernelGGL((join_mfma_kernel<KS>), grid, block, 0, st, fL, fR, volL, volR, C, D, ds, H, W, tiles);             \
	} while (0)
	if (ks <= 56) MC_JOIN_LAUNCH(56);
	else MC_JOIN_LAUNCH(64);
#undef MC_JOIN_LAUNCH
	int rc = check_launch("stereo_join_hwd");
	if (rc || n <= 0) return rc;
	hipLaunchKernelGGL(fix_border_hwd_kernel, dim3(cdiv((int64_t)H * n * 64, 256)), block, 0, st, volL, D, ds, H, W, n, -1);
	hipLaunchKernelGGL(fix_border_hwd_kernel, dim3(cdiv((int64_t)H * n * 64, 256)), block, 0, st, volR, D, ds, H, W, n, 1);
	return check_launch("fix_border_hwd");
}

__global__ void __launch_bounds__(256) census_sig_kernel(const float *__restrict__ img, uint32_t *__restrict__ sig,
                                                         uint32_t *__restrict__ mask, int Cimg, int H, int W)
{
	const int64_t id = (int64_t)blockIdx.x * blockDim.x + threadIdx.x;
	const int64_t HW = (int64_t)H * W;
	if (id >= (int64_t)Cimg * HW) return;
	const int c = (int)(id / HW);
	const int64_t pix = id - c * HW;
	const int x = (int)(pix % W), y = (int)(pix / W);
	const float *__restrict__ im = img + c * HW;
	const float p = im[pix];
	uint32_t s[3] = {0, 0, 0}, m[3] = {0, 0, 0};
	int t = 0;
	for (int yy = y - 4; yy <= y + 4; yy++) {
		for (int xx = x - 4; xx <= x + 4; xx++, t++) {
			if (0 <= xx && xx < W && 0 <= yy && yy < H) {
				m[t >> 5] |= 1u << (t & 31);
				if (im[(int64_t)yy * W + xx] < p) s[t >> 5] |= 1u << (t & 31);
			}
		}
	}
	uint32_t *so = sig + id * 3;
	so[0] = s[0]; so[1] = s[1]; so[2] = s[2];
	if (c == 0) {
		uint32_t *mo = mask + pix * 3;
		mo[0] = m[0]; mo[1] = m[1]; mo[2] = m[2];
	}
}

__global__ void __launch_bounds__(256) census_cost_kernel(const uint32_t *__restrict__ sig0, const uint32_t *__restrict__ sig1,
                                                          const uint32_t *__restrict__ mask, float *__restrict__ out, int Cimg, int D,
                                                          int H, int W, int direction)
{
	const int x = blockIdx.x * 256 + threadIdx.x;
	const int y = blockIdx.y;
	const int d = blockIdx.z * direction;
	if (x >= W) return;
	const int64_t HW = (int64_t)H * W;
	const int64_t pix = (int64_t)y * W + x;
	float dist;
	if (0 <= x + d && x + d < W) {
		const uint32_t *m0 = mask + pix * 3, *m1 = mask + (pix + d) * 3;
		const uint32_t v0 = m0[0] & m1[0], v1 = m0[1] & m1[1], v2 = m0[2] & m1[2];
		const int oob = 81 - (__popc(v0) + __popc(v1) + __popc(v2));
		dist = 0;
		for (int c = 0; c < Cimg; c++) {
			const uint32_t *a = sig0 + (c * HW + pix) * 3, *b = sig1 + (c * HW + pix + d) * 3;
			const int diff = __popc((a[0] ^ b[0]) & v0) + __popc((a[1] ^ b[1]) & v1) + __popc((a[2] ^ b[2]) & v2);
			dist += (float)(oob + diff);
		}
		dist /= (float)Cimg;
	} else {
		dist = __builtin_nanf("");
	}
	out[(int64_t)blockIdx.z * HW + pix] = dist;
}

size_t census_scratch_bytes(int Cimg, int H, int W)
{
	return (((size_t)2 * Cimg + 1) * H * W * 3 * sizeof(uint32_t) + 255) & ~(size_t)255;
}

int census_sig(const float *x0, const float *x1, float *vol, void *scratch, int Cimg, int D, int H, int W, int direction,
               hipStream_t st)
{
	const int64_t HW = (int64_t)H * W;
	uint32_t *s0 = (uint32_t *)scratch, *s1 = s0 + (size_t)Cimg * HW * 3, *mk = s1 + (size_t)Cimg * HW * 3;
	hipLaunchKernelGGL(census_sig_kernel, dim3(cdiv((int64_t)Cimg * HW, 256)), dim3(256), 0, st, x0, s0, mk, Cimg, H, W);
	hipLaunchKernelGGL(census_sig_kernel, dim3(cdiv((int64_t)Cimg * HW, 256)), dim3(256), 0, st, x1, s1, mk, Cimg, H, W);
	hipLaunchKernelGGL(census_cost_kernel, dim3(cdiv(W, 256), H, D), dim3(256), 0, st, s0, s1, mk, vol, Cimg, D, H, W, direction);
	return check_launch("census");
}

__global__ void __launch_bounds__(256) ad_tile_kernel(const float *__restrict__ x0, const float *__restrict__ x1, float *__restrict__ out,
                                                      int D, int H, int W, int direction)
{
	constexpr int TY = 16, TX = 64, R = 4, TS = TX + 2 * R + 1;
	__shared__ float A[(TY + 2 * R) * TS];
	const int bx = blockIdx.x * TX, by = blockIdx.y * TY;
	const int d = blockIdx.z * direction;
	const float NANV = __builtin_nanf("");
	for (int i = threadIdx.x; i < (TY + 2 * R) * (TX + 2 * R); i += 256) {
		const int ty = i / (TX + 2 * R), tx = i - ty * (TX + 2 * R);
		const int yy = by + ty - R, xx = bx + tx - R;
		float v = NANV;
		if (0 <= xx && xx < W && 0 <= xx + d && xx + d < W && 0 <= yy && yy < H) {
			const int64_t ind = (int64_t)yy * W + xx;
			v = fabsf(x0[ind] - x1[ind + d]);
		}
		A[ty * TS + tx] = v;
	}
	__syncthreads();
	const int lx = threadIdx.x & 63, wv = threadIdx.x >> 6;
	const int x = bx + lx;
	if (x >= W) return;
	const int64_t HW = (int64_t)H * W;
	for (int r = wv; r < TY; r += 4) {
		const int y = by + r;
		if (y >= H) break;
		float dist;
		if (0 <= x + d && x + d < W) {
			int cnt = 0;
			dist = 0;
			const float *base = A + r * TS + lx;
#pragma unroll
			for (int j = 0; j < 2 * R + 1; ++j) {
#pragma unroll
				for (int k = 0; k < 2 * R + 1; ++k) {
					const float v = base[j * TS + k];
					const bool ok = v == v;
					dist += ok ? v : -0.0f;
					cnt += ok ? 1 : 0;
				}
			}
			dist /= (float)cnt;
		} else {
			dist = NANV;
		}
		out[(int64_t)blockIdx.z * HW + (int64_t)y * W + x] = dist;
	}
}

int ad_tiled(const float *x0, const float *x1, float *vol, int D, int H, int W, int direction, hipStream_t st)
{
	hipLaunchKernelGGL(ad_tile_kernel, dim3(cdiv(W, 64), cdiv(H, 16), D), dim3(256), 0, st, x0, x1, vol, D, H, W, direction);
	return check_launch("ad");
}

}
```

Baseline: 80130 MPix-disp/s.

## Fuse stereo join with first SGM horizontal sweeps in a per-row line kernel

Adds a line mode to the join kernel. Each wave computes the matching-cost runs for one image row with MFMA into LDS and then immediately runs the horizontal SGM recurrence over them, writing both the cost volume and the first sweep output. The separate horizontal sweep pass in the first SGM iteration is skipped, which saves re-reading the cost volume and one launch. The trade-off is a grid of only H blocks of 4 waves, so parallelism is much lower, and the SGM step is moved into a shared header.

```diff
diff --git a/mc-cnn_amd/csrc/api.hip b/mc-cnn_amd/csrc/api.hip
--- a/mc-cnn_amd/csrc/api.hip
+++ b/mc-cnn_amd/csrc/api.hip
@@ -1,4 +1,5 @@
 #include "cbca_common.h"
+#include "sgm_step.h"
 
 #include <stdarg.h>
 #include <algorithm>
@@ -21,6 +22,8 @@
 int mean2d(const float *img, const float *kernel, float *out, int H, int W, int ks, float alpha2, hipStream_t st);
 int normalize_forward(const float *in, float *norm, float *out, int N, int C, int H, int W, hipStream_t st);
 int stereo_join_dhw(const float *fL, const float *fR, float *volL, float *volR, int C, int D, int H, int W, hipStream_t st);
+bool join_sweep_fits(int C, int D, int ds, int H, int W, int n);
+int stereo_join_sweep_hwd(const float *fL, const float *fR, int C, int H, int W, int n, const SgmPassArgs &S, hipStream_t st);
 int stereo_join_hwd(const float *fL, const float *fR, float *volL, float *volR, int C, int D, int ds, int H, int W, int n,
                     hipStream_t st);
 int ad_tiled(const float *x0, const float *x1, float *vol, int D, int H, int W, int direction, hipStream_t st);
@@ -56,7 +59,7 @@
 int sgm_contract_violations(const float *vol, int H, int W, int D, unsigned *count, hipStream_t st);
 int sgm_sweeps(const float *const C[2], float *const out[2], float *const out2[2], float *const disp[2],
                const int direction[2], int nvol, int H, int W, int D, int ds, const void *maps, float pi1, float pi2,
-               float alpha1, float q1, float q2, bool fused, unsigned drop_final, hipStream_t st);
+               float alpha1, float q1, float q2, bool fused, unsigned drop_final, bool skip_horizontal, hipStream_t st);
 
 static thread_local char g_err[512] = "";
 
@@ -325,8 +328,10 @@
 		return 0;
 	};
 	const bool join_fits = (int64_t)W * ((D + 3) / 4 * 4) * 4 < ((int64_t)1 << 31) && ((int64_t)(C + 64) * HW + W) * 4 < ((int64_t)1 << 31);
+	bool join_sweep = false;
 	if (from_feat && n_cbca1 == 0 && n_sgm > 0 && join_fits) {
-		RUN(stereo_join_hwd(featL, featR, bufA[0], bufA[1], C, D, ds, H, W, p->border_n, st));
+		join_sweep = join_sweep_fits(C, D, ds, H, W, p->border_n);
+		if (!join_sweep) RUN(stereo_join_hwd(featL, featR, bufA[0], bufA[1], C, D, ds, H, W, p->border_n, st));
 		cur[0] = bufA[0]; cur[1] = bufA[1];
 		hwd = true;
 		tm.mark(ST_JOIN);
@@ -364,8 +369,14 @@
 			float *outv[2] = {other(0), other(1)};
 			const bool am = (it == n_sgm - 1) && n_cbca2 == 0;
 			const unsigned drop_final = (am && nvol == 2 && !volR_out) ? 2u : 0u;
+			const bool lines_in_join = join_sweep && it == 0;
+			if (lines_in_join) {
+				SgmPassArgs S;
+				sgm_pass_args(S, Cv, outv, bufC, nullptr, direction, nvol, H, W, D, ds, maps, p->pi1, p->pi2, p->alpha1, p->sgm_q1, p->sgm_q2);
+				RUN(stereo_join_sweep_hwd(featL, featR, C, H, W, p->border_n, S, st));
+			}
 			RUN(sgm_sweeps(Cv, outv, bufC, am ? dispv : nullptr, direction, nvol, H, W, D, ds, maps, p->pi1, p->pi2, p->alpha1,
-			               p->sgm_q1, p->sgm_q2, true, drop_final, st));
+			               p->sgm_q1, p->sgm_q2, true, drop_final, lines_in_join, st));
 			have_disp = am;
 			cur[0] = outv[0]; cur[1] = outv[1];
 		}
@@ -737,7 +748,7 @@
 	const float *Cv[2] = {in_hwd, in_hwd};
 	float *outv[2] = {out_hwd, out_hwd};
 	const int dirv[2] = {direction, direction};
-	return sgm_sweeps(Cv, outv, nullptr, nullptr, dirv, 1, H, W, D, D, tmp, pi1, pi2, alpha1, sgm_q1, sgm_q2, false, 0u, st);
+	return sgm_sweeps(Cv, outv, nullptr, nullptr, dirv, 1, H, W, D, D, tmp, pi1, pi2, alpha1, sgm_q1, sgm_q2, false, 0u, false, st);
 }
 
 int mc_dhw_to_hwd(const float *in, float *out, int D, int H, int W, void *stream)
diff --git a/mc-cnn_amd/csrc/sgm.hip b/mc-cnn_amd/csrc/sgm.hip
--- a/mc-cnn_amd/csrc/sgm.hip
+++ b/mc-cnn_amd/csrc/sgm.hip
@@ -1,29 +1,7 @@
 #include "mc_common.h"
-
-#define MC_SGM_VOL_AUX 2
-#define MC_SGM_ST_AUX MC_SGM_VOL_AUX
+#include "sgm_step.h"
 
 namespace mc {
-
-constexpr int SGM_PADW = 520;
-
-struct SgmPassArgs {
-	const float *C[2];
-	const float *accin[2];
-	const float *accin2[2];
-	float *out[2];
-	float *out2[2];
-	float *disp[2];
-	int drop_out[2];
-	int direction[2];
-	int nvol;
-	int H, W, D, ds;
-	const uint8_t *cls0;
-	int64_t cls_plane;
-	const uint8_t *win;
-	int Wm;
-	float P1[3], P2[3], P1a[3];
-};
 
 __device__ __forceinline__ int cls_of(float v, float tau) { return v < tau ? 0 : (v > tau ? 2 : 1); }
 
@@ -66,8 +44,6 @@
 	win[((int64_t)(1 * 4 + r) * H + y) * Wm + i] = (uint8_t)desc;
 }
 
-typedef unsigned uint4v __attribute__((ext_vector_type(4)));
-
 template <int VPL, int NACC>
 struct StepData {
 	float c[VPL];
@@ -77,37 +53,6 @@
 	unsigned a0;
 };
 
-
-__device__ __forceinline__ float vmin2(float a, float b)
-{
-	float r;
-	asm("v_min_f32 %0, %1, %2" : "=v"(r) : "v"(a), "v"(b));
-	return r;
-}
-__device__ __forceinline__ float vmin3(float a, float b, float c)
-{
-	float r;
-	asm("v_min3_f32 %0, %1, %2, %3" : "=v"(r) : "v"(a), "v"(b), "v"(c));
-	return r;
-}
-__device__ __forceinline__ float wave_min_q(float v)
-{
-	float r;
-	asm volatile("s_nop 1\n\tv_min_f32_dpp %1, %1, %1 quad_perm:[1,0,3,2] row_mask:0xf bank_mask:0xf\n\t"
-	             "s_nop 1\n\tv_min_f32_dpp %1, %1, %1 quad_perm:[2,3,0,1] row_mask:0xf bank_mask:0xf\n\t"
-	             "s_nop 1\n\tv_min_f32_dpp %1, %1, %1 row_half_mirror row_mask:0xf bank_mask:0xf\n\t"
-	             "s_nop 1\n\tv_min_f32_dpp %1, %1, %1 row_mirror row_mask:0xf bank_mask:0xf\n\t"
-	             "s_nop 1\n\tv_min_f32_dpp %1, %1, %1 row_bcast:15 row_mask:0xa bank_mask:0xf\n\t"
-	             "s_nop 1\n\tv_min_f32_dpp %1, %1, %1 row_bcast:31 row_mask:0xc bank_mask:0xf\n\t"
-	             "s_nop 0\n\tv_readlane_b32 %0, %1, 63"
-	             : "=s"(r), "+v"(v));
-	return r;
-}
-
-__device__ __forceinline__ __amdgpu_buffer_rsrc_t pixel_rsrc(const float *base, int64_t elem_off, int bytes)
-{
-	return __builtin_amdgcn_make_buffer_rsrc((void *)(base + elem_off), 0, bytes, 0x00020000);
-}
 
 template <int DIRN, int VPL, int MODE, bool ARGMIN, bool VEC, int U, bool DUAL, bool FAR>
 __device__ __forceinline__ void sgm_line(const SgmPassArgs &A, int wave)
@@ -143,10 +88,7 @@
 	const int sy = dirn == 2 ? 1 : (dirn == 3 ? -1 : 0);
 
 	const int dbase = VPL * lane;
-	const uint8_t *__restrict__ cls0 = A.cls0 + (int64_t)dirn * A.cls_plane;
-	constexpr int WBIAS = 1024;
-	const uint8_t *__restrict__ win = A.win + ((int64_t)((direction > 0 ? 0 : 1) * 4 + dirn) * H) * Wm + SGM_PADW - WBIAS;
-	const int woff = (direction > 0 ? dbase : -dbase - 3) + WBIAS;
+	const int woff = (direction > 0 ? dbase : -dbase - 3) + SGM_WBIAS;
 	const int wq = direction > 0 ? 4 : -4;
 	const int run_bytes = (VEC ? ds : D) * 4;
 
@@ -166,9 +108,9 @@
 	const __amdgpu_buffer_rsrc_t rA = pixel_rsrc(NACC >= 1 ? Ain : Cp, (int64_t)minpix * ds, FAR ? 0 : span);
 	const __amdgpu_buffer_rsrc_t rA2 = pixel_rsrc(NACC >= 2 ? Ain2 : Cp, (int64_t)minpix * ds, FAR ? 0 : span);
 	const __amdgpu_buffer_rsrc_t rO = pixel_rsrc(Out, (int64_t)minpix * ds, (FAR || drop) ? 0 : span);
-	const __amdgpu_buffer_rsrc_t rW = __builtin_amdgcn_make_buffer_rsrc((void *)win, 0, H * Wm + 2 * WBIAS + 64, 0x00020000);
+	const __amdgpu_buffer_rsrc_t rW = sgm_win_rsrc(A, direction, dirn);
 	const int w0 = y0s * Wm + x0s, dw = sy * Wm + sx;
-	const __amdgpu_buffer_rsrc_t rCls = __builtin_amdgcn_make_buffer_rsrc((void *)cls0, 0, H * W, 0x00020000);
+	const __amdgpu_buffer_rsrc_t rCls = sgm_cls_rsrc(A, dirn);
 	const __amdgpu_buffer_rsrc_t rDisp = pixel_rsrc(ARGMIN ? Disp : Out, 0, H * W * 4);
 	unsigned lane_off[VEC ? VPL / 4 : VPL];
 #pragma unroll
@@ -200,26 +142,16 @@
 		load_run(sd.c, Cp, rC, so, pix);
 		if constexpr (NACC >= 1) load_run(sd.a, Ain, rA, so, pix);
 		if constexpr (NACC >= 2) load_run(sd.a2, Ain2, rA2, so, pix);
-		unsigned pk = 0;
-		const unsigned sw = (unsigned)(w0 + s * dw);
-#pragma unroll
-		for (int q = 0; q < VPL / 4; ++q) pk |= (unsigned)__builtin_amdgcn_raw_buffer_load_b8(rW, woff + q * wq, sw, 0) << (8 * q);
-		sd.pk = pk;
-		sd.a0 = __builtin_amdgcn_raw_buffer_load_b8(rCls, 0, (unsigned)(pix0 + s * dp), 0);
+		sd.pk = sgm_load_window<VPL>(rW, woff, wq, (unsigned)(w0 + s * dw));
+		sd.a0 = sgm_load_cls(rCls, (unsigned)(pix0 + s * dp));
 	};
 
 	auto store_step = [&](const float (&o)[VPL], int s) {
 		const int64_t pix = FAR ? (int64_t)(y0s + s * sy) * W + (x0s + s * sx) : 0;
 		const __amdgpu_buffer_rsrc_t r = FAR ? pixel_rsrc(Out, pix * ds, drop ? 0 : run_bytes) : rO;
 		const unsigned soff = FAR ? 0u : c0v + (unsigned)s * c1v;
-		if (VEC) {
-#pragma unroll
-			for (int q = 0; q < VPL / 4; ++q) {
-				uint4v t;
-				t.x = __float_as_uint(o[4 * q + 0]); t.y = __float_as_uint(o[4 * q + 1]);
-				t.z = __float_as_uint(o[4 * q + 2]); t.w = __float_as_uint(o[4 * q + 3]);
-				__builtin_amdgcn_raw_buffer_store_b128(t, r, lane_off[q], soff, MC_SGM_ST_AUX);
-			}
+		if constexpr (VEC) {
+			sgm_store_run_vec<VPL>(o, r, lane_off, soff);
 		} else {
 #pragma unroll
 			for (int j = 0; j < VPL; ++j) __builtin_amdgcn_raw_buffer_store_b32(__float_as_uint(o[j]), r, lane_off[j], soff, 0);
@@ -251,59 +183,11 @@
 	float P1midv = P1mid, P2midv = P2mid, P1amidv = P1amid, INFv = INF;
 	asm volatile("" : "+v"(P1midv), "+v"(P2midv), "+v"(P1amidv), "+v"(INFv));
 	const float zadd = (DUAL && second) ? -0.0f : 0.0f;
+	const SgmPen pen = {P1lo, P2lo, P1alo, P1hi, P2hi, P1ahi, P1midv, P2midv, P1amidv, INFv};
 
 	auto process = [&](const StepData<VPL, NACC> &sd, int s, float *keep = nullptr) {
-		float val[VPL], o[VPL];
-		const int a0 = __builtin_amdgcn_readfirstlane((int)sd.a0);
-		const int amatch = a0 == 1 ? 3 : a0;
-		float P1x, P2x, P1ax = 0.0f;
-		if (DIRN >= 2)
-			asm("s_cmp_eq_u32 %3, 0\n\ts_cselect_b32 %0, %4, %5\n\ts_cselect_b32 %1, %6, %7\n\ts_cselect_b32 %2, %8, %9"
-			    : "=s"(P1x), "=s"(P2x), "=s"(P1ax)
-			    : "s"(a0), "s"(P1lo), "s"(P1hi), "s"(P2lo), "s"(P2hi), "s"(P1alo), "s"(P1ahi)
-			    : "scc");
-		else
-			asm("s_cmp_eq_u32 %2, 0\n\ts_cselect_b32 %0, %3, %4\n\ts_cselect_b32 %1, %5, %6"
-			    : "=s"(P1x), "=s"(P2x)
-			    : "s"(a0), "s"(P1lo), "s"(P1hi), "s"(P2lo), "s"(P2hi)
-			    : "scc");
-		const float down = lane_from_below(prev[VPL - 1], INF);
-		const float up = lane_from_above(prev[0], INF);
-#pragma unroll
-		for (int j = 0; j < VPL; ++j) {
-			const int b = (sd.pk >> (2 * j)) & 3;
-			const bool match = b == amatch;
-			const float P2 = match ? P2x : P2midv;
-			const float P1 = match ? P1x : P1midv;
-			const float P1a = match ? P1ax : P1amidv;
-			const float pm = j > 0 ? prev[j > 0 ? j - 1 : 0] : down;
-			const float pp = j < VPL - 1 ? prev[j < VPL - 1 ? j + 1 : 0] : up;
-			float cost;
-			asm("v_min_f32 %0, %1, %2\n\tv_min3_f32 %0, %0, %3, %4"
-			    : "=&v"(cost)
-			    : "v"(prev[j]), "v"(m + P2), "v"(pm + (DIRN == 2 ? P1a : P1)), "v"(pp + (DIRN == 3 ? P1a : P1)));
-			val[j] = (sd.c[j] + cost) - m;
-		}
-		if (s == 0) {
-			asm volatile("; border step");
-#pragma unroll
-			for (int j = 0; j < VPL; ++j) val[j] = sd.c[j];
-		}
-		float q[VPL];
-#pragma unroll
-		for (int j = 0; j < VPL; ++j) {
-			if (MODE == 0) o[j] = val[j] + zadd;
-			else if (MODE == 1) o[j] = sd.a[j] + val[j];
-			else if (MODE == 2) o[j] = (sd.a[j] + val[j]) * 0.25f;
-			else o[j] = (sd.a[j] + sd.a2[j]) + val[j];
-			q[j] = vmin2(val[j], INFv);
-		}
-#pragma unroll
-		for (int j = 0; j < VPL; ++j) prev[j] = (dbase + j < D) ? q[j] : INFv;
-		float nm = vmin3(prev[0], prev[1], prev[2]);
-#pragma unroll
-		for (int j = 3; j < VPL; j += 2) nm = j + 1 < VPL ? vmin3(nm, prev[j], prev[j + 1]) : vmin2(nm, prev[j]);
-		m = wave_min_q(nm);
+		float o[VPL];
+		sgm_step<DIRN, VPL, MODE>(sd.c, sd.a, sd.a2, sd.pk, sd.a0, s == 0, prev, m, o, pen, zadd, dbase, D);
 		if (keep) {
 #pragma unroll
 			for (int j = 0; j < VPL; ++j) keep[j] = o[j];
@@ -439,12 +323,10 @@
 }
 
 
-int sgm_sweeps(const float *const C[2], float *const out[2], float *const out2[2], float *const disp[2],
-               const int direction[2], int nvol, int H, int W, int D, int ds, const void *maps, float pi1, float pi2,
-               float alpha1, float q1, float q2, bool fused, unsigned drop_final, hipStream_t st)
-{
-	MC_REQUIRE((int64_t)H * W < ((int64_t)1 << 29) && (int64_t)W * ds * 4 < ((int64_t)1 << 31), "sgm: image %dx%d (pixel stride %d) exceeds the sweeps' 32-bit line arithmetic", H, W, ds);
-	SgmPassArgs A;
+void sgm_pass_args(SgmPassArgs &A, const float *const C[2], float *const out[2], float *const out2[2], float *const disp[2],
+                   const int direction[2], int nvol, int H, int W, int D, int ds, const void *maps, float pi1, float pi2,
+                   float alpha1, float q1, float q2)
+{
 	for (int v = 0; v < 2; ++v) {
 		const int k = v < nvol ? v : 0;
 		A.C[v] = C[k];
@@ -466,6 +348,15 @@
 	A.P1[1] = pi1 / q1; A.P2[1] = pi2 / q1;
 	A.P1[2] = pi1 / (q1 * q2); A.P2[2] = pi2 / (q1 * q2);
 	for (int k = 0; k < 3; ++k) A.P1a[k] = A.P1[k] / alpha1;
+}
+
+int sgm_sweeps(const float *const C[2], float *const out[2], float *const out2[2], float *const disp[2],
+               const int direction[2], int nvol, int H, int W, int D, int ds, const void *maps, float pi1, float pi2,
+               float alpha1, float q1, float q2, bool fused, unsigned drop_final, bool skip_horizontal, hipStream_t st)
+{
+	MC_REQUIRE((int64_t)H * W < ((int64_t)1 << 29) && (int64_t)W * ds * 4 < ((int64_t)1 << 31), "sgm: image %dx%d (pixel stride %d) exceeds the sweeps' 32-bit line arithmetic", H, W, ds);
+	SgmPassArgs A;
+	sgm_pass_args(A, C, out, out2, disp, direction, nvol, H, W, D, ds, maps, pi1, pi2, alpha1, q1, q2);
 
 	bool vec = (ds % 4 == 0);
 	for (int v = 0; v < nvol; ++v) {
@@ -480,7 +371,7 @@
 		launch_pass<3, 1, false, false>(A, vec, st);
 	} else {
 		MC_REQUIRE(out2 && vec, "sgm: the fused sweeps need the second direction's scratch and 16-byte aligned volumes with ds %% 4 == 0");
-		launch_pass<0, 0, false, true>(A, vec, st);
+		if (!skip_horizontal) launch_pass<0, 0, false, true>(A, vec, st);
 		launch_pass<2, 3, false, false>(A, vec, st);
 		for (int v = 0; v < nvol; ++v) A.drop_out[v] = (drop_final >> v) & 1;
 		if (am) launch_pass<3, 2, true, false>(A, vec, st);
diff --git a/mc-cnn_amd/csrc/sgm_step.h b/mc-cnn_amd/csrc/sgm_step.h
--- /dev/null
+++ b/mc-cnn_amd/csrc/sgm_step.h
@@ -0,0 +1,165 @@
+#pragma once
+#include "mc_common.h"
+
+#define MC_SGM_VOL_AUX 2
+#define MC_SGM_ST_AUX MC_SGM_VOL_AUX
+
+namespace mc {
+
+constexpr int SGM_PADW = 520;
+constexpr int SGM_WBIAS = 1024;
+
+struct SgmPassArgs {
+	const float *C[2];
+	const float *accin[2];
+	const float *accin2[2];
+	float *out[2];
+	float *out2[2];
+	float *disp[2];
+	int drop_out[2];
+	int direction[2];
+	int nvol;
+	int H, W, D, ds;
+	const uint8_t *cls0;
+	int64_t cls_plane;
+	const uint8_t *win;
+	int Wm;
+	float P1[3], P2[3], P1a[3];
+};
+
+typedef unsigned uint4v __attribute__((ext_vector_type(4)));
+
+__device__ __forceinline__ float vmin2(float a, float b)
+{
+	float r;
+	asm("v_min_f32 %0, %1, %2" : "=v"(r) : "v"(a), "v"(b));
+	return r;
+}
+__device__ __forceinline__ float vmin3(float a, float b, float c)
+{
+	float r;
+	asm("v_min3_f32 %0, %1, %2, %3" : "=v"(r) : "v"(a), "v"(b), "v"(c));
+	return r;
+}
+__device__ __forceinline__ float wave_min_q(float v)
+{
+	float r;
+	asm volatile("s_nop 1\n\tv_min_f32_dpp %1, %1, %1 quad_perm:[1,0,3,2] row_mask:0xf bank_mask:0xf\n\t"
+	             "s_nop 1\n\tv_min_f32_dpp %1, %1, %1 quad_perm:[2,3,0,1] row_mask:0xf bank_mask:0xf\n\t"
+	             "s_nop 1\n\tv_min_f32_dpp %1, %1, %1 row_half_mirror row_mask:0xf bank_mask:0xf\n\t"
+	             "s_nop 1\n\tv_min_f32_dpp %1, %1, %1 row_mirror row_mask:0xf bank_mask:0xf\n\t"
+	             "s_nop 1\n\tv_min_f32_dpp %1, %1, %1 row_bcast:15 row_mask:0xa bank_mask:0xf\n\t"
+	             "s_nop 1\n\tv_min_f32_dpp %1, %1, %1 row_bcast:31 row_mask:0xc bank_mask:0xf\n\t"
+	             "s_nop 0\n\tv_readlane_b32 %0, %1, 63"
+	             : "=s"(r), "+v"(v));
+	return r;
+}
+
+__device__ __forceinline__ __amdgpu_buffer_rsrc_t pixel_rsrc(const float *base, int64_t elem_off, int bytes)
+{
+	return __builtin_amdgcn_make_buffer_rsrc((void *)(base + elem_off), 0, bytes, 0x00020000);
+}
+
+struct SgmPen {
+	float P1lo, P2lo, P1alo, P1hi, P2hi, P1ahi;
+	float P1midv, P2midv, P1amidv, INFv;
+};
+
+__device__ __forceinline__ __amdgpu_buffer_rsrc_t sgm_win_rsrc(const SgmPassArgs &A, int direction, int dirn)
+{
+	const uint8_t *win = A.win + ((int64_t)((direction > 0 ? 0 : 1) * 4 + dirn) * A.H) * A.Wm + SGM_PADW - SGM_WBIAS;
+	return __builtin_amdgcn_make_buffer_rsrc((void *)win, 0, A.H * A.Wm + 2 * SGM_WBIAS + 64, 0x00020000);
+}
+__device__ __forceinline__ __amdgpu_buffer_rsrc_t sgm_cls_rsrc(const SgmPassArgs &A, int dirn)
+{
+	return __builtin_amdgcn_make_buffer_rsrc((void *)(A.cls0 + (int64_t)dirn * A.cls_plane), 0, A.H * A.W, 0x00020000);
+}
+template <int VPL>
+__device__ __forceinline__ unsigned sgm_load_window(const __amdgpu_buffer_rsrc_t &rW, int woff, int wq, unsigned wpix)
+{
+	unsigned pk = 0;
+#pragma unroll
+	for (int q = 0; q < VPL / 4; ++q) pk |= (unsigned)__builtin_amdgcn_raw_buffer_load_b8(rW, woff + q * wq, wpix, 0) << (8 * q);
+	return pk;
+}
+__device__ __forceinline__ unsigned sgm_load_cls(const __amdgpu_buffer_rsrc_t &rCls, unsigned pix)
+{
+	return __builtin_amdgcn_raw_buffer_load_b8(rCls, 0, pix, 0);
+}
+
+template <int VPL>
+__device__ __forceinline__ void sgm_store_run_vec(const float (&o)[VPL], const __amdgpu_buffer_rsrc_t &r, const unsigned (&lane_off)[VPL / 4],
+                                                  unsigned soff)
+{
+#pragma unroll
+	for (int q = 0; q < VPL / 4; ++q) {
+		uint4v t;
+		t.x = __float_as_uint(o[4 * q + 0]); t.y = __float_as_uint(o[4 * q + 1]);
+		t.z = __float_as_uint(o[4 * q + 2]); t.w = __float_as_uint(o[4 * q + 3]);
+		__builtin_amdgcn_raw_buffer_store_b128(t, r, lane_off[q], soff, MC_SGM_ST_AUX);
+	}
+}
+
+template <int DIRN, int VPL, int MODE>
+__device__ __forceinline__ void sgm_step(const float (&c)[VPL], const float *a, const float *a2, unsigned pk, unsigned a0v, bool first,
+                                         float (&prev)[VPL], float &m, float (&o)[VPL], const SgmPen &P, float zadd, int dbase, int D)
+{
+	const float INF = __builtin_inff();
+	float val[VPL];
+	const int a0 = __builtin_amdgcn_readfirstlane((int)a0v);
+	const int amatch = a0 == 1 ? 3 : a0;
+	float P1x, P2x, P1ax = 0.0f;
+	if (DIRN >= 2)
+		asm("s_cmp_eq_u32 %3, 0\n\ts_cselect_b32 %0, %4, %5\n\ts_cselect_b32 %1, %6, %7\n\ts_cselect_b32 %2, %8, %9"
+		    : "=s"(P1x), "=s"(P2x), "=s"(P1ax)
+		    : "s"(a0), "s"(P.P1lo), "s"(P.P1hi), "s"(P.P2lo), "s"(P.P2hi), "s"(P.P1alo), "s"(P.P1ahi)
+		    : "scc");
+	else
+		asm("s_cmp_eq_u32 %2, 0\n\ts_cselect_b32 %0, %3, %4\n\ts_cselect_b32 %1, %5, %6"
+		    : "=s"(P1x), "=s"(P2x)
+		    : "s"(a0), "s"(P.P1lo), "s"(P.P1hi), "s"(P.P2lo), "s"(P.P2hi)
+		    : "scc");
+	const float down = lane_from_below(prev[VPL - 1], INF);
+	const float up = lane_from_above(prev[0], INF);
+#pragma unroll
+	for (int j = 0; j < VPL; ++j) {
+		const int b = (pk >> (2 * j)) & 3;
+		const bool match = b == amatch;
+		const float P2 = match ? P2x : P.P2midv;
+		const float P1 = match ? P1x : P.P1midv;
+		const float P1a = match ? P1ax : P.P1amidv;
+		const float pm = j > 0 ? prev[j > 0 ? j - 1 : 0] : down;
+		const float pp = j < VPL - 1 ? prev[j < VPL - 1 ? j + 1 : 0] : up;
+		float cost;
+		asm("v_min_f32 %0, %1, %2\n\tv_min3_f32 %0, %0, %3, %4"
+		    : "=&v"(cost)
+		    : "v"(prev[j]), "v"(m + P2), "v"(pm + (DIRN == 2 ? P1a : P1)), "v"(pp + (DIRN == 3 ? P1a : P1)));
+		val[j] = (c[j] + cost) - m;
+	}
+	if (first) {
+		asm volatile("; border step");
+#pragma unroll
+		for (int j = 0; j < VPL; ++j) val[j] = c[j];
+	}
+	float q[VPL];
+#pragma unroll
+	for (int j = 0; j < VPL; ++j) {
+		if (MODE == 0) o[j] = val[j] + zadd;
+		else if (MODE == 1) o[j] = a[j] + val[j];
+		else if (MODE == 2) o[j] = (a[j] + val[j]) * 0.25f;
+		else o[j] = (a[j] + a2[j]) + val[j];
+		q[j] = vmin2(val[j], P.INFv);
+	}
+#pragma unroll
+	for (int j = 0; j < VPL; ++j) prev[j] = (dbase + j < D) ? q[j] : P.INFv;
+	float nm = vmin3(prev[0], prev[1], prev[2]);
+#pragma unroll
+	for (int j = 3; j < VPL; j += 2) nm = j + 1 < VPL ? vmin3(nm, prev[j], prev[j + 1]) : vmin2(nm, prev[j]);
+	m = wave_min_q(nm);
+}
+
+void sgm_pass_args(SgmPassArgs &A, const float *const C[2], float *const out[2], float *const out2[2], float *const disp[2],
+                   const int direction[2], int nvol, int H, int W, int D, int ds, const void *maps, float pi1, float pi2,
+                   float alpha1, float q1, float q2);
+
+}
diff --git a/mc-cnn_amd/csrc/stereo_join.hip b/mc-cnn_amd/csrc/stereo_join.hip
--- a/mc-cnn_amd/csrc/stereo_join.hip
+++ b/mc-cnn_amd/csrc/stereo_join.hip
@@ -1,4 +1,5 @@
 #include "mc_common.h"
+#include "sgm_step.h"
 #include <type_traits>
 
 namespace mc {
@@ -288,15 +289,197 @@
 	}
 }
 
+
+typedef float floatx4 __attribute__((ext_vector_type(4)));
+#ifndef MC_JOIN_LINE_DBG
+#define MC_JOIN_LINE_DBG 0
+#endif
+constexpr int JL_PX = 16;
+constexpr int JL_RUN = 256;
+
+template <int KSTEPS>
+__device__ __forceinline__ void join_line(const float *__restrict__ fL, const float *__restrict__ fR, int C, int H, int W,
+                                          const SgmPassArgs &S, int border_n, int y, int v, bool second, float *__restrict__ runs)
+{
+	constexpr int NK = KSTEPS / 2;
+	const int lane = threadIdx.x & 63;
+	const int nl = lane & 15, kq = lane >> 4;
+	const int D = S.D, ds = S.ds;
+	const int64_t HW = (int64_t)H * W;
+	const unsigned feat_bytes = (unsigned)(((int64_t)(C - 1) * HW + W) * 4);
+	const __amdgpu_buffer_rsrc_t rOwn = __builtin_amdgcn_make_buffer_rsrc((void *)((v == 0 ? fL : fR) + (int64_t)y * W), 0, feat_bytes, 0x00020000);
+	const __amdgpu_buffer_rsrc_t rPar = __builtin_amdgcn_make_buffer_rsrc((void *)((v == 0 ? fR : fL) + (int64_t)y * W), 0, feat_bytes, 0x00020000);
+	const unsigned quad_bytes = (unsigned)(4 * HW * 4);
+	constexpr unsigned OOBF = 0x80000000u;
+	const float NANV = __builtin_nanf("");
+	auto load_tile = [&](float (&t)[NK], const __amdgpu_buffer_rsrc_t &r, int px, bool negate) {
+		const unsigned vo = (px >= 0 && px < W) ? (unsigned)((int64_t)kq * HW + px) * 4u : OOBF;
+#pragma unroll
+		for (int kk = 0; kk < NK; ++kk) {
+			const float f = __uint_as_float(__builtin_amdgcn_raw_buffer_load_b32(r, vo + (unsigned)kk * quad_bytes, 0, 0));
+			t[kk] = negate ? -f : f;
+		}
+	};
+	const int bsrc = v == 0 ? W - border_n - 1 : border_n;
+	auto own_pos = [&](int x) { return v == 0 ? min(x, bsrc) : max(x, bsrc); };
+	const int nblk = (W + JL_PX - 1) / JL_PX;
+	auto tiles_of = [&](int k, int &Tlo, int &npairs) {
+		const int lo = own_pos(JL_PX * k), hi = own_pos(min(JL_PX * k + JL_PX - 1, W - 1));
+		Tlo = v == 0 ? (lo - D + 1) >> 4 : lo >> 4;
+		const int Thi = v == 0 ? hi >> 4 : (hi + D - 1) >> 4;
+		npairs = (Thi - Tlo + 2) >> 1;
+	};
+
+	const int dirn = second ? 1 : 0;
+	const int direction = S.direction[v];
+	const int dbase = 4 * lane;
+	const int woff = (direction > 0 ? dbase : -dbase - 3) + SGM_WBIAS;
+	const __amdgpu_buffer_rsrc_t rW = sgm_win_rsrc(S, direction, dirn);
+	const __amdgpu_buffer_rsrc_t rCls = sgm_cls_rsrc(S, dirn);
+	const int row_bytes = W * ds * 4;
+	float *Out = second ? S.out2[v] : S.out[v];
+	const __amdgpu_buffer_rsrc_t rO = pixel_rsrc(Out, (int64_t)y * W * ds, row_bytes);
+	const __amdgpu_buffer_rsrc_t rC = pixel_rsrc(S.C[v], (int64_t)y * W * ds, second ? 0 : row_bytes);
+	constexpr unsigned OOBV = 0x80000000u;
+	unsigned lane_off[1];
+	lane_off[0] = (unsigned)dbase * 4u < (unsigned)(ds * 4) ? (unsigned)dbase * 4u : OOBV;
+	const float INF = __builtin_inff();
+	float P1midv = S.P1[1], P2midv = S.P2[1], P1amidv = S.P1a[1], INFv = INF;
+	asm volatile("" : "+v"(P1midv), "+v"(P2midv), "+v"(P1amidv), "+v"(INFv));
+	const SgmPen pen = {S.P1[0], S.P2[0], S.P1a[0], S.P1[2], S.P2[2], S.P1a[2], P1midv, P2midv, P1amidv, INFv};
+	const float zadd = second ? -0.0f : 0.0f;
+	float prev[4] = {0.0f, 0.0f, 0.0f, 0.0f};
+	float m = 0.0f;
+
+	const int kstep = second ? -1 : 1;
+	int k = second ? nblk - 1 : 0;
+	int Tlo, npairs;
+	tiles_of(k, Tlo, npairs);
+	float own[NK], own_nxt[NK], pa[NK], pb[NK], pc[NK], pd[NK];
+	load_tile(own, rOwn, own_pos(JL_PX * k + nl), true);
+	load_tile(pa, rPar, JL_PX * Tlo + nl, false);
+	load_tile(pb, rPar, JL_PX * (Tlo + 1) + nl, false);
+
+	for (int blk = 0; blk < nblk; ++blk, k += kstep) {
+		const int p0 = JL_PX * k;
+		const int np = min(JL_PX, W - p0);
+		const int kn = blk + 1 < nblk ? k + kstep : k;
+		int Tlo_n, npairs_n;
+		tiles_of(kn, Tlo_n, npairs_n);
+		load_tile(own_nxt, rOwn, own_pos(JL_PX * kn + nl), true);
+		unsigned pk[JL_PX];
+#pragma unroll
+		for (int i = 0; i < JL_PX; ++i) {
+			const int ii = min(i, np - 1);
+			const int x = p0 + (second ? np - 1 - ii : ii);
+			pk[i] = sgm_load_window<4>(rW, woff, 0, (unsigned)(y * S.Wm + x));
+		}
+		unsigned a0all;
+		{
+			const int ii = min(nl, np - 1);
+			const int x = p0 + (second ? np - 1 - ii : ii);
+			a0all = __builtin_amdgcn_raw_buffer_load_b8(rCls, (unsigned)(y * W + x), 0, 0);
+		}
+		int opos[4];
+#pragma unroll
+		for (int r = 0; r < 4; ++r) opos[r] = own_pos(p0 + 4 * kq + r);
+
+		auto put_tile = [&](int T, const floatx4 &acc) {
+			const int pp = JL_PX * T + nl;
+			const bool pin = pp >= 0 && pp < W;
+#pragma unroll
+			for (int r = 0; r < 4; ++r) {
+				const int d = v == 0 ? opos[r] - pp : pp - opos[r];
+				if ((unsigned)d < (unsigned)D) runs[(4 * kq + r) * JL_RUN + d] = pin ? acc[r] : NANV;
+			}
+		};
+		for (int p = 0; p < npairs; ++p) {
+			const int T = Tlo + 2 * p;
+			const int Tn = p + 1 < npairs ? T + 2 : Tlo_n;
+			load_tile(pc, rPar, JL_PX * Tn + nl, false);
+			load_tile(pd, rPar, JL_PX * (Tn + 1) + nl, false);
+			floatx4 acc0 = {0.0f, 0.0f, 0.0f, 0.0f}, acc1 = {0.0f, 0.0f, 0.0f, 0.0f};
+			const bool any_in = JL_PX * T + 2 * JL_PX - 1 >= 0 && JL_PX * T < W;
+			if (any_in && !(MC_JOIN_LINE_DBG & 1)) {
+#pragma unroll
+				for (int kk = 0; kk < NK; ++kk) {
+					acc0 = __builtin_amdgcn_mfma_f32_16x16x4f32(own[kk], pa[kk], acc0, 0, 0, 0);
+					acc1 = __builtin_amdgcn_mfma_f32_16x16x4f32(own[kk], pb[kk], acc1, 0, 0, 0);
+				}
+			}
+			put_tile(T, acc0);
+			put_tile(T + 1, acc1);
+#pragma unroll
+			for (int kk = 0; kk < NK; ++kk) { pa[kk] = pc[kk]; pb[kk] = pd[kk]; }
+		}
+
+		auto consume = [&](auto full_tag) {
+			constexpr bool FULL = decltype(full_tag)::value;
+#pragma unroll
+			for (int g = 0; g < JL_PX; g += 4) {
+				if (!FULL && g >= np) break;
+				float c[4][4], o[4][4];
+#pragma unroll
+				for (int u = 0; u < 4; ++u) {
+					const int i = g + u;
+					const int mrow = second ? np - 1 - i : i;
+					const float4 t = *(const float4 *)(runs + (FULL ? mrow : max(min(mrow, JL_PX - 1), 0)) * JL_RUN + dbase);
+					c[u][0] = t.x; c[u][1] = t.y; c[u][2] = t.z; c[u][3] = t.w;
+				}
+#pragma unroll
+				for (int u = 0; u < 4; ++u) {
+					const int i = g + u;
+					if (FULL || i < np) {
+						const int x = p0 + (second ? np - 1 - i : i);
+						const bool first = second ? x == W - 1 : x == 0;
+						if (MC_JOIN_LINE_DBG & 4) {
+#pragma unroll
+							for (int j = 0; j < 4; ++j) o[u][j] = c[u][j];
+						} else {
+							sgm_step<0, 4, 0>(c[u], nullptr, nullptr, pk[i], (unsigned)__builtin_amdgcn_readlane((int)a0all, i), first, prev, m,
+							                  o[u], pen, zadd, dbase, D);
+						}
+					}
+				}
+				if (!(MC_JOIN_LINE_DBG & 2)) {
+#pragma unroll
+					for (int u = 0; u < 4; ++u) {
+						const int i = g + u;
+						if (FULL || i < np) {
+							const unsigned soff = (unsigned)((p0 + (second ? np - 1 - i : i)) * ds * 4);
+							sgm_store_run_vec<4>(c[u], rC, lane_off, soff);
+							sgm_store_run_vec<4>(o[u], rO, lane_off, soff);
+						}
+					}
+				}
+			}
+		};
+		if (np == JL_PX) consume(std::true_type{});
+		else consume(std::false_type{});
+
+#pragma unroll
+		for (int kk = 0; kk < NK; ++kk) own[kk] = own_nxt[kk];
+		Tlo = Tlo_n;
+		npairs = npairs_n;
+	}
+}
+
 #define MC_JOIN_NT 2
 #define MC_JOIN_WPB 4
 template <int KSTEPS, int NT = MC_JOIN_NT>
 __global__ void __launch_bounds__(64 * MC_JOIN_WPB) join_owner_kernel(const float *__restrict__ fL, const float *__restrict__ fR,
                                                          float *__restrict__ volL, float *__restrict__ volR, int C, int D, int ds,
-                                                         int H, int W, int pairs_per_row)
+                                                         int H, int W, int pairs_per_row, int mode, int border_n, const SgmPassArgs S)
 {
 	__shared__ __attribute__((aligned(16))) float rings[MC_JOIN_WPB][NT * 32 * 64];
 	const int wid = __builtin_amdgcn_readfirstlane(threadIdx.x >> 6);
+	if (mode == 1) {
+		static_assert(NT * 32 * 64 == JL_PX * JL_RUN, "a wave's LDS is one block of runs");
+		const int y = blockIdx.x, v = wid >> 1;
+		if (y >= H || v >= S.nvol) return;
+		join_line<KSTEPS>(fL, fR, C, H, W, S, border_n, y, v, (wid & 1) != 0, rings[wid]);
+		return;
+	}
 	const int b = blockIdx.x;
 	const int xcd = b & 7, k = b >> 3;
 	const int blocks_per_row = (2 * pairs_per_row + MC_JOIN_WPB - 1) / MC_JOIN_WPB;
@@ -331,10 +514,11 @@
 	           "stereo_join_hwd: the volumes must be 16-byte aligned with a pixel stride ds %% 4 == 0 (ds = %d)", ds);
 	if (ks <= 32) {
 		const int tiles_own = ((W + 31) / 32 + MC_JOIN_NT - 1) / MC_JOIN_NT;
+		SgmPassArgs no_sweep = {};
 		const dim3 grid_o((unsigned)(rows8 * ((2 * tiles_own + MC_JOIN_WPB - 1) / MC_JOIN_WPB) * 8)), block_o(64 * MC_JOIN_WPB);
-		if (ks <= 8) hipLaunchKernelGGL((join_owner_kernel<8>), grid_o, block_o, 0, st, fL, fR, volL, volR, C, D, ds, H, W, tiles_own);
-		else if (ks <= 16) hipLaunchKernelGGL((join_owner_kernel<16>), grid_o, block_o, 0, st, fL, fR, volL, volR, C, D, ds, H, W, tiles_own);
-		else hipLaunchKernelGGL((join_owner_kernel<32>), grid_o, block_o, 0, st, fL, fR, volL, volR, C, D, ds, H, W, tiles_own);
+		if (ks <= 8) hipLaunchKernelGGL((join_owner_kernel<8>), grid_o, block_o, 0, st, fL, fR, volL, volR, C, D, ds, H, W, tiles_own, 0, 0, no_sweep);
+		else if (ks <= 16) hipLaunchKernelGGL((join_owner_kernel<16>), grid_o, block_o, 0, st, fL, fR, volL, volR, C, D, ds, H, W, tiles_own, 0, 0, no_sweep);
+		else hipLaunchKernelGGL((join_owner_kernel<32>), grid_o, block_o, 0, st, fL, fR, volL, volR, C, D, ds, H, W, tiles_own, 0, 0, no_sweep);
 		int rc = check_launch("stereo_join_hwd (owner tiles)");
 		if (rc || n <= 0) return rc;
 		hipLaunchKernelGGL(fix_border_hwd_kernel, dim3(cdiv((int64_t)H * n * 64, 256)), block, 0, st, volL, D, ds, H, W, n, -1);
@@ -358,6 +542,26 @@
 	return check_launch("fix_border_hwd");
 }
 
+bool join_sweep_fits(int C, int D, int ds, int H, int W, int n)
+{
+	return C <= 64 && D <= JL_RUN && ds % 4 == 0 && n >= 0 && n < W && (int64_t)H * W * ds * 4 < ((int64_t)1 << 31);
+}
+
+int stereo_join_sweep_hwd(const float *fL, const float *fR, int C, int H, int W, int n, const SgmPassArgs &S, hipStream_t st)
+{
+	MC_REQUIRE(join_sweep_fits(C, S.D, S.ds, H, W, n), "stereo_join_sweep_hwd: C=%d D=%d ds=%d n=%d outside what the line mode covers", C, S.D, S.ds, n);
+	for (int v = 0; v < S.nvol; ++v)
+		MC_REQUIRE((uintptr_t)S.C[v] % 16 == 0 && (uintptr_t)S.out[v] % 16 == 0 && (uintptr_t)S.out2[v] % 16 == 0 && S.direction[v] == (v == 0 ? -1 : 1),
+		           "stereo_join_sweep_hwd: the volumes must be 16-byte aligned, volume 0 the left one");
+	const int ks = (C + 1) / 2;
+	const dim3 grid((unsigned)H), block(64 * MC_JOIN_WPB);
+	float *none = nullptr;
+	if (ks <= 8) hipLaunchKernelGGL((join_owner_kernel<8>), grid, block, 0, st, fL, fR, none, none, C, S.D, S.ds, H, W, 0, 1, n, S);
+	else if (ks <= 16) hipLaunchKernelGGL((join_owner_kernel<16>), grid, block, 0, st, fL, fR, none, none, C, S.D, S.ds, H, W, 0, 1, n, S);
+	else hipLaunchKernelGGL((join_owner_kernel<32>), grid, block, 0, st, fL, fR, none, none, C, S.D, S.ds, H, W, 0, 1, n, S);
+	return check_launch("stereo_join_sweep_hwd");
+}
+
 __global__ void __launch_bounds__(256) census_sig_kernel(const float *__restrict__ img, uint32_t *__restrict__ sig,
                                                          uint32_t *__restrict__ mask, int Cimg, int H, int W)
 {
```

After: 61360 MPix-disp/s. -23.4%, worse.
